# teticio/audio-diffusion

Measured on NVIDIA H100. Metric: mel-spectrograms/sec (1000-step DDPM, 256x256x1), higher is better.
Workload: dtype bf16 operands, fp32 accumulate (fp32 master weights, fp64 GroupNorm sums)

## Files before the change

### audio_diffusion_b200/_lib.py

```python
from __future__ import annotations

import ctypes as C
import os

_HERE = os.path.dirname(os.path.abspath(__file__))
LIB_PATH = os.environ.get("B200AD_LIB") or os.path.join(_HERE, "libb200ad.so")

MAX_BLOCKS = 8


class UNetConfigC(C.Structure):
    _fields_ = [
        ("in_channels", C.c_int), ("out_channels", C.c_int), ("layers_per_block", C.c_int), ("num_blocks", C.c_int),
        ("block_out_channels", C.c_int * MAX_BLOCKS), ("down_attn", C.c_int * MAX_BLOCKS),
        ("up_attn", C.c_int * MAX_BLOCKS), ("norm_num_groups", C.c_int), ("norm_eps", C.c_float),
        ("attention_head_dim", C.c_int), ("cross_attention_dim", C.c_int), ("down_cross", C.c_int * MAX_BLOCKS),
        ("up_cross", C.c_int * MAX_BLOCKS),
    ]


class VAEConfigC(C.Structure):
    _fields_ = [
        ("in_channels", C.c_int), ("out_channels", C.c_int), ("latent_channels", C.c_int), ("layers_per_block", C.c_int),
        ("num_blocks", C.c_int), ("block_out_channels", C.c_int * MAX_BLOCKS), ("norm_num_groups", C.c_int),
        ("norm_eps", C.c_float),
    ]


class OptimHParamsC(C.Structure):
    _fields_ = [("lr", C.c_float), ("beta1", C.c_float), ("beta2", C.c_float), ("eps", C.c_float),
                ("weight_decay", C.c_float), ("max_grad_norm", C.c_float), ("ema_decay", C.c_float), ("step", C.c_int)]


class StepCoefC(C.Structure):
    _fields_ = [("sqrt_1m_at", C.c_float), ("inv_sqrt_at", C.c_float), ("clip", C.c_float), ("c_x0", C.c_float),
                ("c_xt", C.c_float), ("c_eps", C.c_float), ("c_z", C.c_float), ("do_clip", C.c_int)]


class MelConfigC(C.Structure):
    _fields_ = [("x_res", C.c_int), ("y_res", C.c_int), ("sample_rate", C.c_int), ("n_fft", C.c_int),
                ("hop_length", C.c_int), ("top_db", C.c_int), ("n_iter", C.c_int)]


_VP, _SZ, _I = C.c_void_p, C.c_size_t, C.c_int
SYMBOLS = {
    "b200ad_last_error": (C.c_char_p, []),
    "b200ad_version": (_I, []),
    "b200ad_unet_create": (_I, [C.POINTER(UNetConfigC), C.POINTER(_VP)]),
    "b200ad_unet_destroy": (None, [_VP]),
    "b200ad_unet_num_params": (_I, [_VP]),
    "b200ad_unet_param_name": (C.c_char_p, [_VP, _I]),
    "b200ad_unet_param_shape": (_I, [_VP, _I, C.POINTER(C.c_int64)]),
    "b200ad_unet_packed_bytes": (_SZ, [_VP]),
    "b200ad_unet_workspace_bytes": (_SZ, [_VP, _I, _I, _I]),
    "b200ad_unet_set_params": (_I, [_VP, C.POINTER(_VP), _VP, _SZ, _VP]),
    "b200ad_unet_bind_workspace": (_I, [_VP, _VP, _SZ, _I, _I, _I, _VP]),
    "b200ad_unet_forward": (_I, [_VP, _VP, _VP, _VP, _VP]),
    "b200ad_unet_set_encoding": (_I, [_VP, _VP, _I]),
    "b200ad_unet_forward_step": (_I, [_VP, _VP, _VP, _VP, C.POINTER(StepCoefC), _VP, _VP, _VP]),
    "b200ad_unet_forward_step_dev": (_I, [_VP, _VP, _VP, _VP, _VP, _VP, _VP]),
    "b200ad_step_scalars_upload": (_I, [C.POINTER(StepCoefC), C.c_float, _VP, _VP, C.c_int, _VP]),
    "b200ad_unet_profile_step": (_I, [_VP, _VP, _VP, _VP, C.POINTER(StepCoefC), _VP, C.POINTER(C.c_float),
                                      C.POINTER(_I), C.POINTER(C.c_double), _I, _VP]),
    "b200ad_unet_debug_tensor": (_I, [_VP, C.c_char_p, _VP, C.POINTER(_I), _VP]),
    "b200ad_unet_last_launch_count": (_I, [_VP]),
    "b200ad_unet_conv_plan": (_I, [_VP, _I, _I, _I, _I, C.POINTER(_I), _I]),
    "b200ad_unet_set_training": (_I, [_VP, _I]),
    "b200ad_unet_grad_floats": (_SZ, [_VP]),
    "b200ad_unet_grad_offset": (_SZ, [_VP, _I]),
    "b200ad_unet_backward_bytes": (_SZ, [_VP]),
    "b200ad_unet_bind_backward": (_I, [_VP, _VP, _SZ, _VP, _VP]),
    "b200ad_unet_backward": (_I, [_VP, _VP, _VP, _I, _VP]),
    "b200ad_unet_backward_launch_count": (_I, [_VP]),
    "b200ad_unet_debug_grad": (_I, [_VP, C.c_char_p, _I, _VP, C.POINTER(_I), _VP]),
    "b200ad_vae_set_training": (_I, [_VP, _I]),
    "b200ad_vae_grad_floats": (_SZ, [_VP]),
    "b200ad_vae_grad_offset": (_SZ, [_VP, _I]),
    "b200ad_vae_backward_bytes": (_SZ, [_VP]),
    "b200ad_vae_bind_backward": (_I, [_VP, _VP, _SZ, _VP, _VP]),
    "b200ad_vae_decoder_backward": (_I, [_VP, _VP, _VP, _I, _VP]),
    "b200ad_vae_encoder_backward": (_I, [_VP, _VP, _VP, _I, _VP]),
    "b200ad_vae_backward_launch_count": (_I, [_VP]),
    "b200ad_vae_debug_grad": (_I, [_VP, C.c_char_p, _I, _VP, C.POINTER(_I), _VP]),
    "b200ad_vae_create": (_I, [C.POINTER(VAEConfigC), C.POINTER(_VP)]),
    "b200ad_vae_destroy": (None, [_VP]),
    "b200ad_vae_num_params": (_I, [_VP]),
    "b200ad_vae_param_name": (C.c_char_p, [_VP, _I]),
    "b200ad_vae_param_shape": (_I, [_VP, _I, C.POINTER(C.c_int64)]),
    "b200ad_vae_packed_bytes": (_SZ, [_VP]),
    "b200ad_vae_workspace_bytes": (_SZ, [_VP, _I, _I, _I]),
    "b200ad_vae_set_params": (_I, [_VP, C.POINTER(_VP), _VP, _SZ, _VP]),
    "b200ad_vae_bind_workspace": (_I, [_VP, _VP, _SZ, _I, _I, _I, _VP]),
    "b200ad_vae_encode": (_I, [_VP, _VP, _VP, _VP, _VP, _VP]),
    "b200ad_vae_decode": (_I, [_VP, _VP, _VP, _VP]),
    "b200ad_vae_debug_tensor": (_I, [_VP, C.c_char_p, _VP, C.POINTER(_I), _VP]),
    "b200ad_vae_last_launch_count": (_I, [_VP]),
    "b200ad_optim_create": (_I, [_I, C.POINTER(C.c_int64), C.POINTER(_VP), C.POINTER(_VP), C.POINTER(_VP),
                                C.POINTER(_VP), C.POINTER(_VP)]),
    "b200ad_optim_destroy": (None, [_VP]),
    "b200ad_optim_step": (_I, [_VP, C.POINTER(_VP), C.POINTER(OptimHParamsC), _VP, _VP]),
    "b200ad_mse_loss_grad": (_I, [_VP, _VP, _SZ, _VP, _VP, _VP, _VP]),
    "b200ad_conv2d_scratch_bytes": (_SZ, [_I] * 7),
    "b200ad_conv2d": (_I, [_VP] * 7 + [_I] * 7 + [_VP, _SZ, _VP]),
    "b200ad_conv2d_dgrad": (_I, [_VP, _VP, _VP] + [_I] * 6 + [_VP, _SZ, _VP]),
    "b200ad_conv2d_wgrad_scratch_bytes": (_SZ, [_I] * 5),
    "b200ad_conv2d_wgrad": (_I, [_VP, _VP, _VP] + [_I] * 6 + [_VP, _SZ, _VP]),
    "b200ad_gn_conv2d": (_I, [_VP, _VP, _VP, _I, C.c_float, _I, _VP, _VP, _VP] + [_I] * 6 + [_VP, _SZ, _VP]),
    "b200ad_group_norm": (_I, [_VP] * 4 + [_I] * 5 + [C.c_float, _I, _VP, _SZ, _VP]),
    "b200ad_mha_scratch_bytes": (_SZ, [_I] * 5),
    "b200ad_mha_forward_backward": (_I, [_VP] * 8 + [_I] * 5 + [_VP, _SZ, _VP]),
    "b200ad_mel_scratch_bytes": (_SZ, [C.POINTER(MelConfigC), _I]),
    "b200ad_mel_encode": (_I, [C.POINTER(MelConfigC), _VP, _VP, _VP, _I, _VP, _SZ, _VP]),
    "b200ad_mel_encode_ref": (_I, [C.POINTER(MelConfigC), _VP, _VP, _VP, _I, _VP, _VP, _VP, _SZ, _VP]),
    "b200ad_mel_decode": (_I, [C.POINTER(MelConfigC), _VP, _VP, _VP, _I, C.c_uint64, _VP, _SZ, _VP]),
    "b200ad_sample_to_u8": (_I, [_VP, _VP, _SZ, _VP]),
}

_lib = None


def lib() -> C.CDLL:
    global _lib
    if _lib is None:
        if not os.path.exists(LIB_PATH):
            raise RuntimeError(
                f"{LIB_PATH} is missing: build it with `python -c 'import __graft_entry__ as g; g.build()'` "
                "(there is no CPU fallback for the audio_diffusion_b200 hot path)")
        l = C.CDLL(LIB_PATH)
        for name, (res, args) in SYMBOLS.items():
            fn = getattr(l, name)
            fn.restype = res
            fn.argtypes = args
        _lib = l
    return _lib


class B200ADError(RuntimeError):
    pass


def check(status: int) -> None:
    if status != 0:
        raise B200ADError(lib().b200ad_last_error().decode())


def require_cuda():
    import torch

    if not torch.cuda.is_available():
        raise B200ADError("audio_diffusion_b200 needs a CUDA device (H100, sm_90a); there is no CPU fallback")


def stream_ptr():
    import torch

    return C.c_void_p(torch.cuda.current_stream().cuda_stream)
```

### audio_diffusion_b200/csrc/api.cu

```cuda
#include <cstdio>
#include <cstring>

#include "../../include/b200ad.h"
#include "bwd_kernels.cuh"
#include "taps.cuh"

namespace b200ad {
int set_err(const char* fmt, ...);
}
using namespace b200ad;

#define CK(call)                                                                      \
  do {                                                                                \
    cudaError_t e__ = (call);                                                         \
    if (e__ != cudaSuccess) return set_err("%s: %s", #call, cudaGetErrorString(e__)); \
  } while (0)

static size_t al(size_t x) { return (x + 255) & ~(size_t)255; }

struct ConvScratch {
  size_t x, par, res, out, wpack, ident, stats, instats, ss, total;
};
static ConvScratch conv_scratch_layout(int N, int cin, int cout, int H, int W, int K, int stride) {
  ConvScratch s{};
  const Geom gi = make_geom(N, H, W);
  const int Ho = stride > 0 ? H / stride : 2 * H, Wo = stride > 0 ? W / stride : 2 * W;
  const Geom go = make_geom(N, Ho, Wo);
  size_t off = 0;
  s.x = off; off = al(off + (size_t)N * (cin / 8) * gi.PL * 16);
  s.par = off; if (stride == 2) off = al(off + (size_t)4 * N * (cin / 8) * go.PL * 16);
  s.res = off; off = al(off + (size_t)N * (cout / 8) * go.PL * 16);
  s.out = off; off = al(off + (size_t)N * (cout / 8) * go.PL * 16);
  s.wpack = off; off = al(off + (size_t)(cout / 128) * (cin / 16) * (K * K > 16 ? K * K : 16) * CONV_B_TAP);
  s.ident = off; off = al(off + (size_t)(cout / 128) * (cout / 16) * CONV_B_TAP);
  s.stats = off; off = al(off + (size_t)N * (cout / 4) * 2 * sizeof(stat_t));
  s.instats = off; off = al(off + (size_t)N * (cin / 4) * 2 * sizeof(stat_t));
  s.ss = off; off = al(off + (size_t)N * cin * sizeof(float2));
  s.total = off;
  return s;
}

extern "C" size_t b200ad_conv2d_scratch_bytes(int N, int cin, int cout, int H, int W, int K, int stride) {
  return conv_scratch_layout(N, cin, cout, H, W, K, stride).total;
}

static int conv2d_impl(const float* x, const float* w, const float* bias, const float* temb, const float* residual,
                       float* y, float* stats_out, int N, int cin, int cout, int H, int W, int K, int stride,
                       const float* gn_gamma, const float* gn_beta, int gn_groups, float gn_eps, int gn_silu,
                       void* scratch, size_t scratch_bytes, void* stream) {
  if (cin % 16 || cout % 128) return set_err("conv2d: cin %% 16 and cout %% 128 must be 0");
  if (!((K == 3 || K == 1) && (stride == 1 || ((stride == 2 || stride == -2) && K == 3)))) return set_err("conv2d: unsupported K/stride");
  if (stride == -2 && (residual || gn_gamma || temb)) return set_err("conv2d: upsample form takes no residual / GroupNorm / temb");
  if (stride == 2 && (H % 2 || W % 2)) return set_err("conv2d: stride 2 needs even H, W");
  if (stride == 2 && (residual || gn_gamma)) return set_err("conv2d: residual / fused GroupNorm need stride 1");
  const ConvScratch L = conv_scratch_layout(N, cin, cout, H, W, K, stride);
  if (scratch_bytes < L.total) return set_err("conv2d: scratch too small");
  cudaStream_t st = (cudaStream_t)stream;
  uint8_t* sb = (uint8_t*)scratch;
  CK(cudaMemsetAsync(sb, 0, L.total, st));
  const int Ho = stride > 0 ? H / stride : 2 * H, Wo = stride > 0 ? W / stride : 2 * W;
  const Geom go = make_geom(N, Ho, Wo);
  __nv_bfloat16* xp = (__nv_bfloat16*)(sb + L.x);
  __nv_bfloat16* par = (__nv_bfloat16*)(sb + L.par);
  __nv_bfloat16* rp = (__nv_bfloat16*)(sb + L.res);
  __nv_bfloat16* op = (__nv_bfloat16*)(sb + L.out);
  __nv_bfloat16* wp = (__nv_bfloat16*)(sb + L.wpack);
  stat_t* stp = (stat_t*)(sb + L.stats);
  CK(launch_nchw_to_pf8(x, xp, N, cin, H, W, st));
  if (residual) CK(launch_nchw_to_pf8(residual, rp, N, cout, Ho, Wo, st));

  ConvParams p{};
  p.N = N; p.H = Ho; p.W = Wo; p.Wp = go.Wp; p.lead = go.lead; p.PL = go.PL;
  p.cout = cout;
  p.out = op; p.bias = bias; p.temb = temb; p.temb_stride = cout;
  p.stats = stats_out ? stp : nullptr;
  if (stride == 1) {
    const TapSet t = taps_conv(K);
    CK(launch_pack_weights(w, cout, cin, K, K, 0, cin / 16, t.pack, wp, st));
    ConvSeg& s = p.seg[0];
    set_seg(s, xp, cin / 8, cin, H, W, wp, t);
    p.nseg = 1;
    if (gn_gamma) {
      stat_t* ist = (stat_t*)(sb + L.instats);
      float2* ss = (float2*)(sb + L.ss);
      CK(launch_quad_stats(xp, ist, N, cin, H, W, st));
      GnApplyParams g{};
      g.src[0] = xp; g.stats[0] = ist; g.C[0] = cin; g.C[1] = 0; g.gamma = gn_gamma; g.beta = gn_beta;
      g.N = N; g.H = H; g.W = W; g.groups = gn_groups; g.eps = gn_eps;
      CK(launch_gn_finalize(g, ss, st));
      s.ss = ss; s.ss_stride = cin; s.silu = gn_silu;
    }
    if (residual) {
      __nv_bfloat16* ident = (__nv_bfloat16*)(sb + L.ident);
      CK(launch_pack_identity(cout, ident, st));
      set_seg(p.seg[1], rp, cout / 8, cout, Ho, Wo, ident, taps_conv(1));
      p.nseg = 2;
    }
  } else if (stride == 2) {
    CK(launch_parity_split(xp, par, N, cin, H, W, st));
    const size_t tsz = (size_t)N * (cin / 8) * go.PL * 8;
    size_t woff = 0;
    for (int a = 0; a < 2; ++a)
      for (int b = 0; b < 2; ++b) {
        const TapSet t = taps_parity(a, b);
        __nv_bfloat16* wseg = wp + woff / 2;
        CK(launch_pack_weights(w, cout, cin, 3, 3, 0, cin / 16, t.pack, wseg, st));
        woff += (size_t)(cout / 128) * (cin / 16) * t.pack.ntaps * CONV_B_TAP;
        set_seg(p.seg[a * 2 + b], par + (size_t)(a * 2 + b) * tsz, cin / 8, cin, Ho, Wo, wseg, t);
      }
    p.nseg = 4;
  }
  int dev = 0, sms = 132;
  CK(cudaGetDevice(&dev));
  CK(cudaDeviceGetAttribute(&sms, cudaDevAttrMultiProcessorCount, dev));
  if (stride == -2) {
    const Geom gi = make_geom(N, H, W);
    p.H = H; p.W = W; p.Wp = gi.Wp; p.lead = gi.lead; p.PL = gi.PL;
    p.up2 = 1;
    p.nseg = 1;
    size_t woff = 0;
    for (int pa = 0; pa < 2; ++pa)
      for (int pb = 0; pb < 2; ++pb) {
        const TapSet t = taps_up2(pa, pb);
        __nv_bfloat16* wseg = wp + woff / 2;
        CK(launch_pack_weights(w, cout, cin, 3, 3, 0, cin / 16, t.pack, wseg, st));
        woff += (size_t)(cout / 128) * (cin / 16) * 4 * CONV_B_TAP;
        set_seg(p.seg[0], xp, cin / 8, cin, H, W, wseg, t);
        p.oy = pa; p.ox = pb;
        CK(launch_conv_tc(p, sms, st));
      }
  } else {
    CK(launch_conv_tc(p, sms, st));
  }
  CK(launch_pf8_to_nchw(op, y, N, cout, Ho, Wo, st));
  if (stats_out) CK(launch_stats_to_float(stp, stats_out, N * (cout / 4) * 2, st));
  return 0;
}

extern "C" int b200ad_conv2d(const float* x, const float* w, const float* bias, const float* temb, const float* residual,
                             float* y, float* stats_out, int N, int cin, int cout, int H, int W, int K, int stride,
                             void* scratch, size_t scratch_bytes, void* stream) {
  return conv2d_impl(x, w, bias, temb, residual, y, stats_out, N, cin, cout, H, W, K, stride, nullptr, nullptr, 0, 0.f, 0,
                     scratch, scratch_bytes, stream);
}

extern "C" int b200ad_conv2d_dgrad(const float* gy, const float* w, float* gx, int N, int cin, int cout, int H, int W, int K,
                                   void* scratch, size_t scratch_bytes, void* stream) {
  if (cout % 16 || cin % 128) return set_err("conv2d_dgrad: cout %% 16 and cin %% 128 must be 0");
  if (K != 3 && K != 1) return set_err("conv2d_dgrad: K must be 1 or 3");
  const ConvScratch L = conv_scratch_layout(N, cout, cin, H, W, K, 1);
  if (scratch_bytes < L.total) return set_err("conv2d_dgrad: scratch too small");
  cudaStream_t st = (cudaStream_t)stream;
  uint8_t* sb = (uint8_t*)scratch;
  CK(cudaMemsetAsync(sb, 0, L.total, st));
  const Geom g = make_geom(N, H, W);
  __nv_bfloat16* gyp = (__nv_bfloat16*)(sb + L.x);
  __nv_bfloat16* gxp = (__nv_bfloat16*)(sb + L.out);
  __nv_bfloat16* wp = (__nv_bfloat16*)(sb + L.wpack);
  CK(launch_nchw_to_pf8(gy, gyp, N, cout, H, W, st));
  const TapSet t = taps_mirrored(K);
  CK(launch_pack_weights(w, cin, cin, K, K, 0, cout / 16, t.pack, wp, st, cin));
  ConvParams p{};
  p.N = N; p.H = H; p.W = W; p.Wp = g.Wp; p.lead = g.lead; p.PL = g.PL;
  p.cout = cin;
  p.out = gxp; p.bias = nullptr; p.temb = nullptr; p.temb_stride = 0; p.stats = nullptr;
  set_seg(p.seg[0], gyp, cout / 8, cout, H, W, wp, t);
  p.nseg = 1;
  int dev = 0, sms = 132;
  CK(cudaGetDevice(&dev));
  CK(cudaDeviceGetAttribute(&sms, cudaDevAttrMultiProcessorCount, dev));
  CK(launch_conv_tc(p, sms, st));
  CK(launch_pf8_to_nchw(gxp, gx, N, cin, H, W, st));
  return 0;
}

extern "C" int b200ad_conv2d_wgrad(const float* gy, const float* a, float* dw, int N, int cin, int cout, int H, int W, int K,
                                   void* scratch, size_t scratch_bytes, void* stream) {
  if (cout % 128 || cin % 32) return set_err("conv2d_wgrad: cout %% 128 and cin %% 32 must be 0");
  if (K != 3 && K != 1) return set_err("conv2d_wgrad: K must be 1 or 3");
  const Geom g = make_geom(N, H, W);
  const size_t gyb = al((size_t)N * (cout / 8) * g.PL * 16), ab = al((size_t)N * (cin / 8) * g.PL * 16);
  if (scratch_bytes < gyb + ab) return set_err("conv2d_wgrad: scratch too small (%zu < %zu)", scratch_bytes, gyb + ab);
  cudaStream_t st = (cudaStream_t)stream;
  uint8_t* sb = (uint8_t*)scratch;
  CK(cudaMemsetAsync(sb, 0, gyb + ab, st));
  __nv_bfloat16* gyp = (__nv_bfloat16*)sb;
  __nv_bfloat16* ap = (__nv_bfloat16*)(sb + gyb);
  CK(launch_nchw_to_pf8(gy, gyp, N, cout, H, W, st));
  CK(launch_nchw_to_pf8(a, ap, N, cin, H, W, st));
  CK(cudaMemsetAsync(dw, 0, (size_t)cout * cin * K * K * sizeof(float), st));
  int dev = 0, sms = 132;
  CK(cudaGetDevice(&dev));
  CK(cudaDeviceGetAttribute(&sms, cudaDevAttrMultiProcessorCount, dev));
  WgradDesc d{};
  d.gy = gyp; d.act = ap; d.dw = dw; d.N = N; d.H = H; d.W = W; d.cout = cout; d.cin = cin;
  d.gy_img_planes = cout / 8; d.act_img_planes = cin / 8; d.cin_total = cin; d.ci_off = 0; d.ntaps_total = K * K;
  const TapSet t = taps_conv(K);
  d.ntaps = K * K;
  for (int k = 0; k < K * K; ++k) { d.dh[k] = t.dh[k]; d.dw_[k] = t.dw[k]; d.tapidx[k] = t.wtap[k]; }
  CK(launch_wgrad_tc(d, sms, st));
  return 0;
}
extern "C" size_t b200ad_conv2d_wgrad_scratch_bytes(int N, int cin, int cout, int H, int W) {
  const Geom g = make_geom(N, H, W);
  return al((size_t)N * (cout / 8) * g.PL * 16) + al((size_t)N * (cin / 8) * g.PL * 16);
}

extern "C" int b200ad_gn_conv2d(const float* x, const float* gamma, const float* beta, int groups, float eps, int silu,
                                const float* w, const float* bias, float* y, int N, int cin, int cout, int H, int W, int K,
                                void* scratch, size_t scratch_bytes, void* stream) {
  if (!gamma || !beta) return set_err("gn_conv2d: gamma and beta are required");
  return conv2d_impl(x, w, bias, nullptr, nullptr, y, nullptr, N, cin, cout, H, W, K, 1, gamma, beta, groups, eps, silu,
                     scratch, scratch_bytes, stream);
}

extern "C" int b200ad_group_norm(const float* x, const float* gamma, const float* beta, float* y, int N, int C, int H,
                                 int W, int groups, float eps, int silu, void* scratch, size_t scratch_bytes, void* stream) {
  if (C % 32) return set_err("group_norm: C %% 32 != 0");
  const Geom g = make_geom(N, H, W);
  const size_t tb = al((size_t)N * (C / 8) * g.PL * 16);
  const size_t need = 2 * tb + al((size_t)N * (C / 4) * 2 * sizeof(stat_t));
  if (scratch_bytes < need) return set_err("group_norm: scratch too small (%zu < %zu)", scratch_bytes, need);
  cudaStream_t st = (cudaStream_t)stream;
  uint8_t* sb = (uint8_t*)scratch;
  CK(cudaMemsetAsync(sb, 0, need, st));
  __nv_bfloat16* xp = (__nv_bfloat16*)sb;
  __nv_bfloat16* yp = (__nv_bfloat16*)(sb + tb);
  stat_t* stats = (stat_t*)(sb + 2 * tb);
  CK(launch_nchw_to_pf8(x, xp, N, C, H, W, st));
  CK(launch_quad_stats(xp, stats, N, C, H, W, st));
  GnApplyParams p{};
  p.src[0] = xp; p.stats[0] = stats; p.C[0] = C; p.src[1] = nullptr; p.stats[1] = nullptr; p.C[1] = 0;
  p.gamma = gamma; p.beta = beta; p.dst = yp; p.N = N; p.H = H; p.W = W; p.groups = groups; p.eps = eps; p.silu = silu;
  CK(launch_gn_apply(p, st));
  CK(launch_pf8_to_nchw(yp, y, N, C, H, W, st));
  return 0;
}

struct MhaScratch {
  size_t qkv_f, qkv, o, go, gqkv, lse, dsum, total;
};
static MhaScratch mha_scratch_layout(int N, int C, int heads, int H, int W) {
  MhaScratch s{};
  const Geom g = make_geom(N, H, W);
  const size_t pf = (size_t)N * (C / 8) * g.PL * 16, rows = (size_t)N * heads * H * W * sizeof(float);
  size_t off = 0;
  s.qkv_f = off; off = al(off + (size_t)N * 3 * C * H * W * sizeof(float));
  s.qkv = off; off = al(off + 3 * pf);
  s.o = off; off = al(off + pf);
  s.go = off; off = al(off + pf);
  s.gqkv = off; off = al(off + 3 * pf);
  s.lse = off; off = al(off + rows);
  s.dsum = off; off = al(off + rows);
  s.total = off;
  return s;
}
extern "C" size_t b200ad_mha_scratch_bytes(int N, int C, int heads, int H, int W) {
  return mha_scratch_layout(N, C, heads, H, W).total;
}
extern "C" int b200ad_mha_forward_backward(const float* q, const float* k, const float* v, const float* dout, float* out,
                                           float* dq, float* dk, float* dv, int N, int C, int heads, int H, int W,
                                           void* scratch, size_t scratch_bytes, void* stream) {
  if (heads < 1 || C % heads || (C / heads != 16 && C / heads != 32 && C / heads != 64))
    return set_err("mha_forward_backward: head_dim C / heads must be 16, 32 or 64");
  const MhaScratch L = mha_scratch_layout(N, C, heads, H, W);
  if (scratch_bytes < L.total) return set_err("mha_forward_backward: scratch too small (%zu < %zu)", scratch_bytes, L.total);
  cudaStream_t st = (cudaStream_t)stream;
  uint8_t* sb = (uint8_t*)scratch;
  CK(cudaMemsetAsync(sb, 0, L.total, st));
  float* qkvf = (float*)(sb + L.qkv_f);
  __nv_bfloat16* qkv = (__nv_bfloat16*)(sb + L.qkv);
  __nv_bfloat16* o = (__nv_bfloat16*)(sb + L.o);
  __nv_bfloat16* go = (__nv_bfloat16*)(sb + L.go);
  __nv_bfloat16* gqkv = (__nv_bfloat16*)(sb + L.gqkv);
  const size_t img = (size_t)C * H * W * sizeof(float);
  const float* src[3] = {q, k, v};
  for (int j = 0; j < 3; ++j)
    CK(cudaMemcpy2DAsync((uint8_t*)qkvf + j * img, 3 * img, src[j], img, img, N, cudaMemcpyDeviceToDevice, st));
  CK(launch_nchw_to_pf8(qkvf, qkv, N, 3 * C, H, W, st));
  CK(launch_nchw_to_pf8(dout, go, N, C, H, W, st));
  CK(launch_mha_flash(qkv, o, N, C, heads, H, W, st, (float*)(sb + L.lse)));
  CK(launch_mha_bwd(qkv, o, go, (const float*)(sb + L.lse), (float*)(sb + L.dsum), gqkv, N, C, heads, H, W, st));
  CK(launch_pf8_to_nchw(o, out, N, C, H, W, st));
  CK(launch_pf8_to_nchw(gqkv, qkvf, N, 3 * C, H, W, st));
  float* dst[3] = {dq, dk, dv};
  for (int j = 0; j < 3; ++j)
    CK(cudaMemcpy2DAsync(dst[j], img, (const uint8_t*)qkvf + j * img, 3 * img, img, N, cudaMemcpyDeviceToDevice, st));
  return 0;
}

extern "C" int b200ad_sample_to_u8(const float* x, uint8_t* img, size_t n, void* stream) {
  CK(launch_sample_to_u8(x, img, n, (cudaStream_t)stream));
  return 0;
}
```

### audio_diffusion_b200/csrc/common.cuh

```cuda
#pragma once
#include <cuda_bf16.h>
#include <cuda_runtime.h>
#include <stdint.h>
#include <stdio.h>

namespace b200ad {

typedef double stat_t;

struct Geom {
  int N, H, W, Wp, lead, PL;
};
__host__ __device__ inline Geom make_geom(int N, int H, int W) {
  Geom g;
  g.N = N; g.H = H; g.W = W; g.Wp = W + 1; g.lead = g.Wp + 8;
  g.PL = g.lead + H * g.Wp + g.Wp + 8 + 512;
  return g;
}

#ifdef __CUDACC__
__device__ __forceinline__ uint32_t smem_u32(const void* p) {
  return static_cast<uint32_t>(__cvta_generic_to_shared(p));
}
__device__ __forceinline__ void mbar_init(uint32_t bar, uint32_t count) {
  asm volatile("mbarrier.init.shared::cta.b64 [%0], %1;" ::"r"(bar), "r"(count));
}
__device__ __forceinline__ void mbar_fence_init() {
  asm volatile("fence.mbarrier_init.release.cluster;" ::: "memory");
}
__device__ __forceinline__ void mbar_arrive_expect_tx(uint32_t bar, uint32_t bytes) {
  asm volatile("mbarrier.arrive.expect_tx.shared::cta.b64 _, [%0], %1;" ::"r"(bar), "r"(bytes) : "memory");
}
__device__ __forceinline__ void mbar_arrive(uint32_t bar) {
  asm volatile("mbarrier.arrive.shared::cta.b64 _, [%0];" ::"r"(bar) : "memory");
}
__device__ __forceinline__ bool mbar_try_wait(uint32_t bar, uint32_t parity) {
  uint32_t ok;
  asm volatile(
      "{\n\t.reg .pred p;\n\t"
      "mbarrier.try_wait.parity.shared::cta.b64 p, [%1], %2;\n\t"
      "selp.u32 %0, 1, 0, p;\n\t}"
      : "=r"(ok) : "r"(bar), "r"(parity) : "memory");
  return ok != 0;
}
__device__ __forceinline__ void mbar_wait(uint32_t bar, uint32_t parity) {
  if (mbar_try_wait(bar, parity)) return;
  long long t0 = clock64();
  while (!mbar_try_wait(bar, parity)) {
    if (clock64() - t0 > 4000000000LL) __trap();
  }
}

__device__ __forceinline__ void mbar_wait_warp(uint32_t bar, uint32_t parity) {
  if (__all_sync(0xffffffffu, mbar_try_wait(bar, parity))) return;
  long long t0 = clock64();
  while (!__all_sync(0xffffffffu, mbar_try_wait(bar, parity))) {
    if (clock64() - t0 > 4000000000LL) {
      if ((threadIdx.x & 31) == 0) printf("b200ad: mbarrier timeout (block %d warp %d bar %u parity %u)\n", blockIdx.x, threadIdx.x >> 5, bar, parity);
      __trap();
    }
  }
}

__device__ __forceinline__ void bulk_g2s(uint32_t dst_smem, const void* src, uint32_t bytes, uint32_t bar) {
  asm volatile(
      "cp.async.bulk.shared::cluster.global.mbarrier::complete_tx::bytes [%0], [%1], %2, [%3];"
      ::"r"(dst_smem), "l"(src), "r"(bytes), "r"(bar) : "memory");
}

__device__ __forceinline__ void bulk_s2g(void* dst, uint32_t src_smem, uint32_t bytes) {
  asm volatile("cp.async.bulk.global.shared::cta.bulk_group [%0], [%1], %2;" ::"l"(dst), "r"(src_smem), "r"(bytes) : "memory");
}
__device__ __forceinline__ void bulk_commit() { asm volatile("cp.async.bulk.commit_group;" ::: "memory"); }
__device__ __forceinline__ void bulk_wait_read_all() { asm volatile("cp.async.bulk.wait_group.read 0;" ::: "memory"); }
__device__ __forceinline__ void bulk_wait_all() { asm volatile("cp.async.bulk.wait_group 0;" ::: "memory"); }
__device__ __forceinline__ void named_bar_sync(int id, int nthreads) {
  asm volatile("bar.sync %0, %1;" ::"r"(id), "r"(nthreads) : "memory");
}

__device__ __forceinline__ void tensor_g2s_5d(uint32_t dst_smem, const void* tmap, int c0, int c1, int c2, int c3, int c4,
                                              uint32_t bar) {
  asm volatile(
      "cp.async.bulk.tensor.5d.shared::cluster.global.tile.mbarrier::complete_tx::bytes [%0], [%1, {%2, %3, %4, %5, %6}], [%7];"
      ::"r"(dst_smem), "l"(tmap), "r"(c0), "r"(c1), "r"(c2), "r"(c3), "r"(c4), "r"(bar) : "memory");
}
__device__ __forceinline__ void tensor_s2g_5d(const void* tmap, int c0, int c1, int c2, int c3, int c4, uint32_t src_smem) {
  asm volatile("cp.async.bulk.tensor.5d.global.shared::cta.tile.bulk_group [%0, {%1, %2, %3, %4, %5}], [%6];"
               ::"l"(tmap), "r"(c0), "r"(c1), "r"(c2), "r"(c3), "r"(c4), "r"(src_smem) : "memory");
}

__device__ __forceinline__ void tensor_g2s_4d(uint32_t dst_smem, const void* tmap, int c0, int c1, int c2, int c3, uint32_t bar) {
  asm volatile(
      "cp.async.bulk.tensor.4d.shared::cluster.global.tile.mbarrier::complete_tx::bytes [%0], [%1, {%2, %3, %4, %5}], [%6];"
      ::"r"(dst_smem), "l"(tmap), "r"(c0), "r"(c1), "r"(c2), "r"(c3), "r"(bar) : "memory");
}
__device__ __forceinline__ void tensor_s2g_4d(const void* tmap, int c0, int c1, int c2, int c3, uint32_t src_smem) {
  asm volatile("cp.async.bulk.tensor.4d.global.shared::cta.tile.bulk_group [%0, {%1, %2, %3, %4}], [%5];"
               ::"l"(tmap), "r"(c0), "r"(c1), "r"(c2), "r"(c3), "r"(src_smem) : "memory");
}

__device__ __forceinline__ void bulk_prefetch_l2(const void* src, uint32_t bytes) {
  asm volatile("cp.async.bulk.prefetch.L2.global [%0], %1;" ::"l"(src), "r"(bytes) : "memory");
}

__device__ __forceinline__ uint64_t gmma_desc(uint32_t saddr, uint32_t lbo_bytes, uint32_t sbo_bytes) {
  uint64_t d = 0;
  d |= (uint64_t)((saddr >> 4) & 0x3FFF);
  d |= (uint64_t)((lbo_bytes >> 4) & 0x3FFF) << 16;
  d |= (uint64_t)((sbo_bytes >> 4) & 0x3FFF) << 32;
  return d;
}
__device__ __forceinline__ void wgmma_fence() { asm volatile("wgmma.fence.sync.aligned;" ::: "memory"); }
__device__ __forceinline__ void wgmma_commit() { asm volatile("wgmma.commit_group.sync.aligned;" ::: "memory"); }
template <int N>
__device__ __forceinline__ void wgmma_wait() { asm volatile("wgmma.wait_group.sync.aligned %0;" ::"n"(N) : "memory"); }

template <int TA, int TB>
__device__ __forceinline__ void wgmma_m64n32k16(float* d, uint64_t a, uint64_t b) {
  asm volatile(
      "{\n\t.reg .pred p;\n\tsetp.ne.b32 p, %18, 0;\n\t"
      "wgmma.mma_async.sync.aligned.m64n32k16.f32.bf16.bf16 {"
      "%0, %1, %2, %3, %4, %5, %6, %7, %8, %9, %10, %11, %12, %13, %14, %15"
      "}, %16, %17, p, 1, 1, %19, %20;\n\t}"
      : "+f"(d[0]), "+f"(d[1]), "+f"(d[2]), "+f"(d[3]), "+f"(d[4]), "+f"(d[5]), "+f"(d[6]), "+f"(d[7]),
        "+f"(d[8]), "+f"(d[9]), "+f"(d[10]), "+f"(d[11]), "+f"(d[12]), "+f"(d[13]), "+f"(d[14]), "+f"(d[15])
      : "l"(a), "l"(b), "r"(1), "n"(TA), "n"(TB));
}
template <int TA, int TB>
__device__ __forceinline__ void wgmma_m64n64k16(float* d, uint64_t a, uint64_t b) {
  asm volatile(
      "{\n\t.reg .pred p;\n\tsetp.ne.b32 p, %34, 0;\n\t"
      "wgmma.mma_async.sync.aligned.m64n64k16.f32.bf16.bf16 {"
      "%0, %1, %2, %3, %4, %5, %6, %7, %8, %9, %10, %11, %12, %13, %14, %15, "
      "%16, %17, %18, %19, %20, %21, %22, %23, %24, %25, %26, %27, %28, %29, %30, %31"
      "}, %32, %33, p, 1, 1, %35, %36;\n\t}"
      : "+f"(d[0]), "+f"(d[1]), "+f"(d[2]), "+f"(d[3]), "+f"(d[4]), "+f"(d[5]), "+f"(d[6]), "+f"(d[7]),
        "+f"(d[8]), "+f"(d[9]), "+f"(d[10]), "+f"(d[11]), "+f"(d[12]), "+f"(d[13]), "+f"(d[14]), "+f"(d[15]),
        "+f"(d[16]), "+f"(d[17]), "+f"(d[18]), "+f"(d[19]), "+f"(d[20]), "+f"(d[21]), "+f"(d[22]), "+f"(d[23]),
        "+f"(d[24]), "+f"(d[25]), "+f"(d[26]), "+f"(d[27]), "+f"(d[28]), "+f"(d[29]), "+f"(d[30]), "+f"(d[31])
      : "l"(a), "l"(b), "r"(1), "n"(TA), "n"(TB));
}
template <int TA, int TB>
__device__ __forceinline__ void wgmma_m64n128k16(float* d, uint64_t a, uint64_t b) {
  asm volatile(
      "{\n\t.reg .pred p;\n\tsetp.ne.b32 p, %66, 0;\n\t"
      "wgmma.mma_async.sync.aligned.m64n128k16.f32.bf16.bf16 {"
      "%0, %1, %2, %3, %4, %5, %6, %7, %8, %9, %10, %11, %12, %13, %14, %15, "
      "%16, %17, %18, %19, %20, %21, %22, %23, %24, %25, %26, %27, %28, %29, %30, %31, "
      "%32, %33, %34, %35, %36, %37, %38, %39, %40, %41, %42, %43, %44, %45, %46, %47, "
      "%48, %49, %50, %51, %52, %53, %54, %55, %56, %57, %58, %59, %60, %61, %62, %63"
      "}, %64, %65, p, 1, 1, %67, %68;\n\t}"
      : "+f"(d[0]), "+f"(d[1]), "+f"(d[2]), "+f"(d[3]), "+f"(d[4]), "+f"(d[5]), "+f"(d[6]), "+f"(d[7]),
        "+f"(d[8]), "+f"(d[9]), "+f"(d[10]), "+f"(d[11]), "+f"(d[12]), "+f"(d[13]), "+f"(d[14]), "+f"(d[15]),
        "+f"(d[16]), "+f"(d[17]), "+f"(d[18]), "+f"(d[19]), "+f"(d[20]), "+f"(d[21]), "+f"(d[22]), "+f"(d[23]),
        "+f"(d[24]), "+f"(d[25]), "+f"(d[26]), "+f"(d[27]), "+f"(d[28]), "+f"(d[29]), "+f"(d[30]), "+f"(d[31]),
        "+f"(d[32]), "+f"(d[33]), "+f"(d[34]), "+f"(d[35]), "+f"(d[36]), "+f"(d[37]), "+f"(d[38]), "+f"(d[39]),
        "+f"(d[40]), "+f"(d[41]), "+f"(d[42]), "+f"(d[43]), "+f"(d[44]), "+f"(d[45]), "+f"(d[46]), "+f"(d[47]),
        "+f"(d[48]), "+f"(d[49]), "+f"(d[50]), "+f"(d[51]), "+f"(d[52]), "+f"(d[53]), "+f"(d[54]), "+f"(d[55]),
        "+f"(d[56]), "+f"(d[57]), "+f"(d[58]), "+f"(d[59]), "+f"(d[60]), "+f"(d[61]), "+f"(d[62]), "+f"(d[63])
      : "l"(a), "l"(b), "r"(1), "n"(TA), "n"(TB));
}
template <int TA, int TB>
__device__ __forceinline__ void wgmma_m64n256k16(float* d, uint64_t a, uint64_t b) {
  asm volatile(
      "{\n\t.reg .pred p;\n\tsetp.ne.b32 p, %130, 0;\n\t"
      "wgmma.mma_async.sync.aligned.m64n256k16.f32.bf16.bf16 {"
      "%0, %1, %2, %3, %4, %5, %6, %7, %8, %9, %10, %11, %12, %13, %14, %15, "
      "%16, %17, %18, %19, %20, %21, %22, %23, %24, %25, %26, %27, %28, %29, %30, %31, "
      "%32, %33, %34, %35, %36, %37, %38, %39, %40, %41, %42, %43, %44, %45, %46, %47, "
      "%48, %49, %50, %51, %52, %53, %54, %55, %56, %57, %58, %59, %60, %61, %62, %63, "
      "%64, %65, %66, %67, %68, %69, %70, %71, %72, %73, %74, %75, %76, %77, %78, %79, "
      "%80, %81, %82, %83, %84, %85, %86, %87, %88, %89, %90, %91, %92, %93, %94, %95, "
      "%96, %97, %98, %99, %100, %101, %102, %103, %104, %105, %106, %107, %108, %109, %110, %111, "
      "%112, %113, %114, %115, %116, %117, %118, %119, %120, %121, %122, %123, %124, %125, %126, %127"
      "}, %128, %129, p, 1, 1, %131, %132;\n\t}"
      : "+f"(d[0]), "+f"(d[1]), "+f"(d[2]), "+f"(d[3]), "+f"(d[4]), "+f"(d[5]), "+f"(d[6]), "+f"(d[7]),
        "+f"(d[8]), "+f"(d[9]), "+f"(d[10]), "+f"(d[11]), "+f"(d[12]), "+f"(d[13]), "+f"(d[14]), "+f"(d[15]),
        "+f"(d[16]), "+f"(d[17]), "+f"(d[18]), "+f"(d[19]), "+f"(d[20]), "+f"(d[21]), "+f"(d[22]), "+f"(d[23]),
        "+f"(d[24]), "+f"(d[25]), "+f"(d[26]), "+f"(d[27]), "+f"(d[28]), "+f"(d[29]), "+f"(d[30]), "+f"(d[31]),
        "+f"(d[32]), "+f"(d[33]), "+f"(d[34]), "+f"(d[35]), "+f"(d[36]), "+f"(d[37]), "+f"(d[38]), "+f"(d[39]),
        "+f"(d[40]), "+f"(d[41]), "+f"(d[42]), "+f"(d[43]), "+f"(d[44]), "+f"(d[45]), "+f"(d[46]), "+f"(d[47]),
        "+f"(d[48]), "+f"(d[49]), "+f"(d[50]), "+f"(d[51]), "+f"(d[52]), "+f"(d[53]), "+f"(d[54]), "+f"(d[55]),
        "+f"(d[56]), "+f"(d[57]), "+f"(d[58]), "+f"(d[59]), "+f"(d[60]), "+f"(d[61]), "+f"(d[62]), "+f"(d[63]),
        "+f"(d[64]), "+f"(d[65]), "+f"(d[66]), "+f"(d[67]), "+f"(d[68]), "+f"(d[69]), "+f"(d[70]), "+f"(d[71]),
        "+f"(d[72]), "+f"(d[73]), "+f"(d[74]), "+f"(d[75]), "+f"(d[76]), "+f"(d[77]), "+f"(d[78]), "+f"(d[79]),
        "+f"(d[80]), "+f"(d[81]), "+f"(d[82]), "+f"(d[83]), "+f"(d[84]), "+f"(d[85]), "+f"(d[86]), "+f"(d[87]),
        "+f"(d[88]), "+f"(d[89]), "+f"(d[90]), "+f"(d[91]), "+f"(d[92]), "+f"(d[93]), "+f"(d[94]), "+f"(d[95]),
        "+f"(d[96]), "+f"(d[97]), "+f"(d[98]), "+f"(d[99]), "+f"(d[100]), "+f"(d[101]), "+f"(d[102]), "+f"(d[103]),
        "+f"(d[104]), "+f"(d[105]), "+f"(d[106]), "+f"(d[107]), "+f"(d[108]), "+f"(d[109]), "+f"(d[110]), "+f"(d[111]),
        "+f"(d[112]), "+f"(d[113]), "+f"(d[114]), "+f"(d[115]), "+f"(d[116]), "+f"(d[117]), "+f"(d[118]), "+f"(d[119]),
        "+f"(d[120]), "+f"(d[121]), "+f"(d[122]), "+f"(d[123]), "+f"(d[124]), "+f"(d[125]), "+f"(d[126]), "+f"(d[127])
      : "l"(a), "l"(b), "r"(1), "n"(TA), "n"(TB));
}
__device__ __forceinline__ void wgmma_m64n128k16_x2(float* d, uint64_t a, uint64_t b0, uint64_t b1) {
  asm volatile(
      "{\n\t.reg .pred p;\n\tsetp.ne.b32 p, %131, 0;\n\t"
      "wgmma.mma_async.sync.aligned.m64n128k16.f32.bf16.bf16 {"
      "%0, %1, %2, %3, %4, %5, %6, %7, %8, %9, %10, %11, %12, %13, %14, %15, "
      "%16, %17, %18, %19, %20, %21, %22, %23, %24, %25, %26, %27, %28, %29, %30, %31, "
      "%32, %33, %34, %35, %36, %37, %38, %39, %40, %41, %42, %43, %44, %45, %46, %47, "
      "%48, %49, %50, %51, %52, %53, %54, %55, %56, %57, %58, %59, %60, %61, %62, %63"
      "}, %128, %129, p, 1, 1, 0, 0;\n\t"
      "wgmma.mma_async.sync.aligned.m64n128k16.f32.bf16.bf16 {"
      "%64, %65, %66, %67, %68, %69, %70, %71, %72, %73, %74, %75, %76, %77, %78, %79, "
      "%80, %81, %82, %83, %84, %85, %86, %87, %88, %89, %90, %91, %92, %93, %94, %95, "
      "%96, %97, %98, %99, %100, %101, %102, %103, %104, %105, %106, %107, %108, %109, %110, %111, "
      "%112, %113, %114, %115, %116, %117, %118, %119, %120, %121, %122, %123, %124, %125, %126, %127"
      "}, %128, %130, p, 1, 1, 0, 0;\n\t}"
      : "+f"(d[0]), "+f"(d[1]), "+f"(d[2]), "+f"(d[3]), "+f"(d[4]), "+f"(d[5]), "+f"(d[6]), "+f"(d[7]),
        "+f"(d[8]), "+f"(d[9]), "+f"(d[10]), "+f"(d[11]), "+f"(d[12]), "+f"(d[13]), "+f"(d[14]), "+f"(d[15]),
        "+f"(d[16]), "+f"(d[17]), "+f"(d[18]), "+f"(d[19]), "+f"(d[20]), "+f"(d[21]), "+f"(d[22]), "+f"(d[23]),
        "+f"(d[24]), "+f"(d[25]), "+f"(d[26]), "+f"(d[27]), "+f"(d[28]), "+f"(d[29]), "+f"(d[30]), "+f"(d[31]),
        "+f"(d[32]), "+f"(d[33]), "+f"(d[34]), "+f"(d[35]), "+f"(d[36]), "+f"(d[37]), "+f"(d[38]), "+f"(d[39]),
        "+f"(d[40]), "+f"(d[41]), "+f"(d[42]), "+f"(d[43]), "+f"(d[44]), "+f"(d[45]), "+f"(d[46]), "+f"(d[47]),
        "+f"(d[48]), "+f"(d[49]), "+f"(d[50]), "+f"(d[51]), "+f"(d[52]), "+f"(d[53]), "+f"(d[54]), "+f"(d[55]),
        "+f"(d[56]), "+f"(d[57]), "+f"(d[58]), "+f"(d[59]), "+f"(d[60]), "+f"(d[61]), "+f"(d[62]), "+f"(d[63]),
        "+f"(d[64]), "+f"(d[65]), "+f"(d[66]), "+f"(d[67]), "+f"(d[68]), "+f"(d[69]), "+f"(d[70]), "+f"(d[71]),
        "+f"(d[72]), "+f"(d[73]), "+f"(d[74]), "+f"(d[75]), "+f"(d[76]), "+f"(d[77]), "+f"(d[78]), "+f"(d[79]),
        "+f"(d[80]), "+f"(d[81]), "+f"(d[82]), "+f"(d[83]), "+f"(d[84]), "+f"(d[85]), "+f"(d[86]), "+f"(d[87]),
        "+f"(d[88]), "+f"(d[89]), "+f"(d[90]), "+f"(d[91]), "+f"(d[92]), "+f"(d[93]), "+f"(d[94]), "+f"(d[95]),
        "+f"(d[96]), "+f"(d[97]), "+f"(d[98]), "+f"(d[99]), "+f"(d[100]), "+f"(d[101]), "+f"(d[102]), "+f"(d[103]),
        "+f"(d[104]), "+f"(d[105]), "+f"(d[106]), "+f"(d[107]), "+f"(d[108]), "+f"(d[109]), "+f"(d[110]), "+f"(d[111]),
        "+f"(d[112]), "+f"(d[113]), "+f"(d[114]), "+f"(d[115]), "+f"(d[116]), "+f"(d[117]), "+f"(d[118]), "+f"(d[119]),
        "+f"(d[120]), "+f"(d[121]), "+f"(d[122]), "+f"(d[123]), "+f"(d[124]), "+f"(d[125]), "+f"(d[126]), "+f"(d[127])
      : "l"(a), "l"(b0), "l"(b1), "r"(1));
}

__device__ __forceinline__ bool elect_one() {
  uint32_t pred;
  asm volatile(
      "{\n\t.reg .pred p;\n\t"
      "elect.sync _|p, 0xffffffff;\n\t"
      "selp.u32 %0, 1, 0, p;\n\t}"
      : "=r"(pred));
  return pred != 0;
}

__device__ __forceinline__ void fence_proxy_async_smem() { asm volatile("fence.proxy.async.shared::cta;" ::: "memory"); }

__device__ __forceinline__ float tanh_approx(float x) {
  float y;
  asm("tanh.approx.f32 %0, %1;" : "=f"(y) : "f"(x));
  return y;
}
__device__ __forceinline__ float silu_tanh(float x) { return x * fmaf(0.5f, tanh_approx(0.5f * x), 0.5f); }
__device__ __forceinline__ float silu_f(float x) { return x / (1.0f + __expf(-x)); }
__device__ __forceinline__ uint32_t pack_bf16x2(float lo, float hi) {
  __nv_bfloat162 v = __floats2bfloat162_rn(lo, hi);
  return *reinterpret_cast<uint32_t*>(&v);
}
__device__ __forceinline__ float2 unpack_bf16x2(uint32_t u) {
  __nv_bfloat162 v = *reinterpret_cast<__nv_bfloat162*>(&u);
  return __bfloat1622float2(v);
}

typedef float2 f32x2_t;
__device__ __forceinline__ f32x2_t f2_pack(float lo, float hi) { return make_float2(lo, hi); }
__device__ __forceinline__ float2 f2_unpack(f32x2_t v) { return v; }
__device__ __forceinline__ f32x2_t f2_add(f32x2_t a, f32x2_t b) { return make_float2(a.x + b.x, a.y + b.y); }
__device__ __forceinline__ f32x2_t f2_fma(f32x2_t a, f32x2_t b, f32x2_t c) {
  return make_float2(fmaf(a.x, b.x, c.x), fmaf(a.y, b.y, c.y));
}
__device__ __forceinline__ f32x2_t f2_from_bf16x2(uint32_t u) {
  return f2_pack(__uint_as_float(u << 16), __uint_as_float(u & 0xffff0000u));
}
__device__ __forceinline__ uint32_t f2_to_bf16x2(f32x2_t v) {
  uint32_t r;
  asm("cvt.rn.bf16x2.f32 %0, %1, %2;" : "=r"(r) : "f"(v.y), "f"(v.x));
  return r;
}

__device__ __forceinline__ void stmatrix_x4_trans(uint32_t saddr, uint32_t r0, uint32_t r1, uint32_t r2, uint32_t r3) {
  asm volatile("stmatrix.sync.aligned.m8n8.x4.trans.shared.b16 [%0], {%1, %2, %3, %4};"
               ::"r"(saddr), "r"(r0), "r"(r1), "r"(r2), "r"(r3) : "memory");
}

__device__ __forceinline__ void mma_bf16_16x8x16(float (&c)[4], uint32_t a0, uint32_t a1, uint32_t a2, uint32_t a3, uint32_t b0,
                                                 uint32_t b1) {
  asm volatile("mma.sync.aligned.m16n8k16.row.col.f32.bf16.bf16.f32 {%0,%1,%2,%3}, {%4,%5,%6,%7}, {%8,%9}, {%0,%1,%2,%3};"
               : "+f"(c[0]), "+f"(c[1]), "+f"(c[2]), "+f"(c[3]) : "r"(a0), "r"(a1), "r"(a2), "r"(a3), "r"(b0), "r"(b1));
}

__device__ __forceinline__ long long pf8_pixel(const Geom& g, int p, int W) {
  return (long long)(g.lead + (p / W) * g.Wp + (p % W)) * 8;
}
#endif

}
```

### audio_diffusion_b200/csrc/conv_tc.cu

```cuda
#include <cuda.h>
#include <cudaTypedefs.h>

#include <cstdlib>

#include "conv_tc.cuh"

namespace b200ad {

struct alignas(64) ConvMaps {
  CUtensorMap src[CONV_MAXSEG];
  CUtensorMap out;
};

__host__ __device__ __forceinline__ int window_pixels(const ConvParams& p, const ConvSeg& sg, int G) {
  return p.tile2d ? (p.tw + sg.hl + sg.hr) * (p.th + sg.ht + sg.hb)
                  : G * CONV_TM + (sg.ht + sg.hb) * p.Wp + sg.hl + sg.hr;
}
__host__ __device__ __forceinline__ int window_pitch(const ConvParams& p, const ConvSeg& sg) {
  return p.tile2d ? p.tw + sg.hl + sg.hr : p.Wp;
}

constexpr int CONV_THREADS = 384;
constexpr int CONV_XF_THREADS = 64;
constexpr int CONV_SPLANE = CONV_MAXG * CONV_TM * 16;
constexpr int CONV_STG_WG = 8 * CONV_SPLANE;
constexpr int CONV_STAGING = 2 * CONV_STG_WG;
static size_t conv_smem_bytes(const ConvParams& p) {
  return (size_t)p.as * p.a_stage + (size_t)p.bs * CONV_B_SLOT + CONV_STAGING + 1024;
}

struct WorkItem {
  int n, ntile, m0, G;
  int r0, c0;
};

__device__ __forceinline__ WorkItem decode_work(const ConvParams& p, int w) {
  WorkItem wi;
  wi.ntile = w % p.ntiles_n;
  const int gidx = w / p.ntiles_n;
  if (p.tile2d) {
    wi.n = gidx / p.groups_per_img;
    const int t = gidx - wi.n * p.groups_per_img, tx = t / p.tiles_y;
    wi.r0 = (t - tx * p.tiles_y) * p.th;
    wi.c0 = tx * p.tw;
    wi.m0 = 0;
    wi.G = CONV_MAXG;
    return wi;
  }
  wi.r0 = wi.c0 = 0;
  if (p.pack) {
    wi.n = gidx * p.pack;
    wi.m0 = 0;
    wi.G = min(p.pack, p.N - wi.n);
    return wi;
  }
  wi.n = gidx / p.groups_per_img;
  const int g = gidx - wi.n * p.groups_per_img;
  wi.m0 = g * (CONV_MAXG * CONV_TM);
  const int rem = p.H * p.Wp - wi.m0;
  wi.G = min(CONV_MAXG, (rem + CONV_TM - 1) / CONV_TM);
  return wi;
}

template <bool SILU>
__device__ __forceinline__ uint4 xform_vec(uint4 v, const f32x2_t (&sc)[4], const f32x2_t (&sh)[4]) {
  uint32_t u[4] = {v.x, v.y, v.z, v.w};
#pragma unroll
  for (int e = 0; e < 4; ++e) {
    f32x2_t a = f2_fma(f2_from_bf16x2(u[e]), sc[e], sh[e]);
    if (SILU) {
      const float2 f = f2_unpack(a);
      a = f2_fma(a, f2_pack(tanh_approx(f.x), tanh_approx(f.y)), a);
    }
    u[e] = f2_to_bf16x2(a);
  }
  return make_uint4(u[0], u[1], u[2], u[3]);
}

template <bool SQUARE>
__global__ void __launch_bounds__(CONV_THREADS, 1) conv_tc_kernel(const __grid_constant__ ConvParams p,
                                                                  const __grid_constant__ ConvMaps maps) {
  constexpr int ASM = CONV_AS_MAX, BSM = CONV_BS_MAX;
  const int AS = p.as;
  const int BS = p.bs;
  extern __shared__ __align__(128) uint8_t smem[];
  const int warp = __shfl_sync(0xffffffffu, (int)(threadIdx.x >> 5), 0);
  const int lane = threadIdx.x & 31;
  const int a_bytes = p.a_stage;

  uint8_t* bring = smem + AS * a_bytes;
  uint8_t* stg = bring + BS * CONV_B_SLOT;
  uint8_t* ctrl = stg + CONV_STAGING;
  uint64_t* bars = reinterpret_cast<uint64_t*>(ctrl);
  const uint32_t smem_base = smem_u32(smem);
  const uint32_t bring_base = smem_u32(bring);
  const uint32_t bar_fullA = smem_u32(bars);
  const uint32_t bar_readyA = smem_u32(bars + ASM);
  const uint32_t bar_emptyA = smem_u32(bars + 2 * ASM);
  const uint32_t bar_fullB = smem_u32(bars + 3 * ASM);
  const uint32_t bar_emptyB = smem_u32(bars + 3 * ASM + BSM);
  static_assert((3 * ASM + 2 * BSM) * 8 <= 1024, "barrier block overflows");

  if (warp == 1 && lane == 0) {
    for (int s = 0; s < AS; ++s) {
      mbar_init(bar_fullA + 8 * s, 1);
      mbar_init(bar_readyA + 8 * s, CONV_XF_THREADS / 32);
      mbar_init(bar_emptyA + 8 * s, 8);
    }
    for (int s = 0; s < BS; ++s) {
      mbar_init(bar_fullB + 8 * s, 1);
      mbar_init(bar_emptyB + 8 * s, 8);
    }
    mbar_fence_init();
  }
  __syncthreads();

  asm volatile("griddepcontrol.launch_dependents;" ::: "memory");
  if (warp != 1) asm volatile("griddepcontrol.wait;" ::: "memory");

  if (warp == 0) {
    int stage = 0;
    uint32_t phase = 0;
    for (int w = blockIdx.x; w < p.total_work; w += gridDim.x) {
      const WorkItem wi = decode_work(p, w);
      for (int s = 0; s < p.nseg; ++s) {
        const ConvSeg& sg = p.seg[s];
        const uint32_t row_bytes = (uint32_t)window_pixels(p, sg, wi.G) * 16u;
        for (int ks = 0; ks < sg.ksteps; ++ks) {
          const uint32_t full = bar_fullA + 8 * stage;
          if (lane == 0) {
            mbar_wait(bar_emptyA + 8 * stage, phase ^ 1);
            mbar_arrive_expect_tx(full, 2u * row_bytes);
          }
          __syncwarp();
          const long long plane = (long long)(2 * ks + (lane & 1)) * p.PL;
          if (p.tile2d) {
            if (lane == 0)
              tensor_g2s_4d(smem_base + stage * a_bytes, &maps.src[s], 8 * (wi.c0 - sg.hl), wi.r0 - sg.ht, 2 * ks, wi.n, full);
          } else if (!p.pack) {
            const int pix0 = p.lead + wi.m0 - sg.ht * p.Wp - sg.hl;
            if (lane < 2)
              bulk_g2s(smem_base + stage * a_bytes + (uint32_t)lane * row_bytes,
                       sg.src + (long long)wi.n * sg.img_stride + (plane + pix0) * 8, row_bytes, full);
          } else {
            const int g = lane >> 1, lead_px = sg.ht * p.Wp + sg.hl, trail_px = sg.hb * p.Wp + sg.hr;
            const int cnt = CONV_TM + (g == 0 ? lead_px : 0) + (g == wi.G - 1 ? trail_px : 0);
            const int doff = (g == 0) ? 0 : lead_px + g * CONV_TM;
            const int pix0 = p.lead - (g == 0 ? lead_px : 0);
            if (g < wi.G && lane < 2 * CONV_MAXG)
              bulk_g2s(smem_base + stage * a_bytes + (uint32_t)(lane & 1) * row_bytes + (uint32_t)doff * 16u,
                       sg.src + (long long)(wi.n + g) * sg.img_stride + (plane + pix0) * 8, (uint32_t)cnt * 16u, full);
          }
          if (++stage == AS) { stage = 0; phase ^= 1; }
        }
      }
    }
  } else if (warp == 1) {
    if (lane == 0) {
      int stage = 0;
      uint32_t phase = 0;
      for (int w = blockIdx.x; w < p.total_work; w += gridDim.x) {
        const int ntile = w % p.ntiles_n;
        for (int s = 0; s < p.nseg; ++s) {
          const ConvSeg& sg = p.seg[s];
          const char* src = reinterpret_cast<const char*>(sg.wpack + (long long)ntile * sg.wtile_stride);
          for (int ks = 0; ks < sg.ksteps; ++ks) {
            for (int t0 = 0; t0 < sg.ntaps; t0 += CONV_BT) {
              const uint32_t bytes = (uint32_t)min(CONV_BT, sg.ntaps - t0) * CONV_B_TAP;
              mbar_wait(bar_emptyB + 8 * stage, phase ^ 1);
              if (p.dbg & 32) {
                mbar_arrive(bar_fullB + 8 * stage);
              } else {
                mbar_arrive_expect_tx(bar_fullB + 8 * stage, bytes);
                bulk_g2s(bring_base + stage * CONV_B_SLOT, src, bytes, bar_fullB + 8 * stage);
              }
              src += bytes;
              if (++stage == BS) { stage = 0; phase ^= 1; }
            }
          }
        }
      }
    }
  } else if (warp >= 4) {
    const int cw = (warp - 4) >> 2, wq = warp & 3, tid = threadIdx.x & 127;
    const uint32_t stg_w = smem_u32(stg) + (uint32_t)(cw * CONV_STG_WG);
    const uint32_t st_addr = stg_w + (uint32_t)((2 * wq + ((lane >> 3) & 1)) * CONV_SPLANE + (8 * (lane >> 4) + (lane & 7)) * 16);
    const Geom og = make_geom(p.N, p.up2 ? 2 * p.H : p.H, p.up2 ? 2 * p.W : p.W);
    const long long out_img_stride = (long long)(p.cout >> 3) * og.PL * 8;
    const int hw_end = p.H * p.Wp;
    const bool do_stats = p.stats != nullptr;
    const bool issuer = tid < 8 * CONV_MAXG;
    float acc[CONV_MAXG * CONV_TM / 2];
    int sa = 0, sb = 0;
    uint32_t pa = 0, pb = 0;
    for (int w = blockIdx.x; w < p.total_work; w += gridDim.x) {
      const WorkItem wi = decode_work(p, w);
#pragma unroll
      for (int i = 0; i < CONV_MAXG * CONV_TM / 2; ++i) acc[i] = 0.f;
      int pend_b = -1, pend_a = -1;
      auto release = [&]() {
        __syncwarp();
        if (lane == 0) {
          if (pend_b >= 0) mbar_arrive(bar_emptyB + 8 * pend_b);
          if (pend_a >= 0) mbar_arrive(bar_emptyA + 8 * pend_a);
        }
      };
      for (int s = 0, ks = 0; s < p.nseg;) {
        const ConvSeg& sg = p.seg[s];
        const uint32_t xlbo = (uint32_t)window_pixels(p, sg, wi.G) * 16u;
        const uint32_t xsbo = p.tile2d ? (uint32_t)window_pitch(p, sg) * 16u : 128u;
        const int ntaps = sg.ntaps;
        mbar_wait(bar_readyA + 8 * sa, pa);
        const uint32_t abase = smem_base + sa * a_bytes;
        for (int t0 = 0; t0 < ntaps; t0 += CONV_BT) {
          mbar_wait(bar_fullB + 8 * sb, pb);
          const uint32_t bbase = bring_base + sb * CONV_B_SLOT + (uint32_t)(cw * 1024);
          const int nt = min(CONV_BT, ntaps - t0);
          wgmma_fence();
          for (int t = 0; t < nt; ++t) {
            const uint64_t wdesc = gmma_desc(bbase + (uint32_t)t * CONV_B_TAP, (CONV_NT / 8) * 128, 128);
            const uint64_t xdesc = gmma_desc(abase + (uint32_t)sg.aoff[t0 + t] * 16u, xlbo, xsbo);
            if constexpr (SQUARE) {
              wgmma_m64n128k16_x2(acc, wdesc, xdesc, xdesc + (128u >> 4));
            } else if (wi.G == 2) {
              wgmma_m64n256k16<0, 0>(acc, wdesc, xdesc);
            } else {
              wgmma_m64n128k16<0, 0>(acc, wdesc, xdesc);
            }
          }
          wgmma_commit();
          wgmma_wait<1>();
          release();
          pend_b = sb;
          pend_a = (t0 + CONV_BT >= ntaps) ? sa : -1;
          if (++sb == BS) { sb = 0; pb ^= 1; }
        }
        if (++sa == AS) { sa = 0; pa ^= 1; }
        if (++ks == sg.ksteps) { ks = 0; ++s; }
      }
      wgmma_wait<0>();
      release();

      if (issuer) bulk_wait_read_all();
      named_bar_sync(1 + cw, 128);
      if (!(p.dbg & 8)) {
        float ssum[2] = {0.f, 0.f}, ssq[2] = {0.f, 0.f};
#pragma unroll
        for (int g = 0; g < CONV_MAXG; ++g) {
          if (g < wi.G) {
            const int n = p.pack ? wi.n + g : wi.n;
            float bias[2];
#pragma unroll
            for (int h = 0; h < 2; ++h) {
              const int c = wi.ntile * CONV_NT + cw * 64 + wq * 16 + 8 * h + (lane >> 2);
              bias[h] = p.bias ? __ldg(p.bias + c) : 0.f;
              if (p.temb) bias[h] += __ldg(p.temb + (long long)n * p.temb_stride + c);
            }
            int m = (p.pack ? 0 : wi.m0 + g * CONV_TM) + 2 * (lane & 3);
            int col = m % p.Wp;
#pragma unroll
            for (int k = 0; k < CONV_TM / 16; ++k) {
              uint32_t pk[4];
#pragma unroll
              for (int u = 0; u < 2; ++u) {
                const int col1 = (col + 1 == p.Wp) ? 0 : col + 1;
                const bool v0 = p.tile2d || (m < hw_end && col < p.W), v1 = p.tile2d || (m + 1 < hw_end && col1 < p.W);
#pragma unroll
                for (int h = 0; h < 2; ++h) {
                  const int j = g * (CONV_TM / 8) + 2 * k + u;
                  const float a0 = v0 ? acc[4 * j + 2 * h] + bias[h] : 0.f;
                  const float a1 = v1 ? acc[4 * j + 2 * h + 1] + bias[h] : 0.f;
                  ssum[h] += a0 + a1;
                  ssq[h] = fmaf(a0, a0, fmaf(a1, a1, ssq[h]));
                  pk[2 * u + h] = pack_bf16x2(a0, a1);
                }
                m += 8;
                col += 8;
                while (col >= p.Wp) col -= p.Wp;
              }
              stmatrix_x4_trans(st_addr + (uint32_t)((g * CONV_TM + 16 * k) * 16), pk[0], pk[1], pk[2], pk[3]);
            }
            if (do_stats && (p.pack || g == wi.G - 1)) {
#pragma unroll
              for (int h = 0; h < 2; ++h) {
                float s1 = ssum[h], s2 = ssq[h];
#pragma unroll
                for (int o = 1; o < 16; o <<= 1) {
                  s1 += __shfl_xor_sync(0xffffffffu, s1, o);
                  s2 += __shfl_xor_sync(0xffffffffu, s2, o);
                }
                if ((lane & 15) == 0) {
                  const int c = wi.ntile * CONV_NT + cw * 64 + wq * 16 + 8 * h + (lane >> 2);
                  stat_t* sdst = p.stats + ((long long)n * (p.cout >> 2) + (c >> 2)) * 2;
                  atomicAdd(sdst, (stat_t)s1);
                  atomicAdd(sdst + 1, (stat_t)s2);
                }
                ssum[h] = 0.f;
                ssq[h] = 0.f;
              }
            }
          }
        }
      }
      if (p.tile2d) {
        fence_proxy_async_smem();
        named_bar_sync(1 + cw, 128);
        if (SQUARE) {
          const int g = tid >> 3, pl = tid & 7;
          if (issuer && !(p.dbg & 2)) {
            const uint32_t src = stg_w + (uint32_t)(pl * CONV_SPLANE + g * CONV_TM * 16);
            const int c = wi.c0 + 8 * g, plane = wi.ntile * 16 + cw * 8 + pl;
            if (p.up2) tensor_s2g_5d(&maps.out, 0, c, wi.r0, plane, wi.n, src);
            else       tensor_s2g_4d(&maps.out, 8 * c, wi.r0, plane, wi.n, src);
            bulk_commit();
          }
        } else if (tid == 0 && !(p.dbg & 2)) {
          tensor_s2g_4d(&maps.out, 8 * wi.c0, wi.r0, wi.ntile * 16 + cw * 8, wi.n, stg_w);
          bulk_commit();
        }
      } else if (!p.up2) {
        fence_proxy_async_smem();
        named_bar_sync(1 + cw, 128);
        const int g = tid >> 3, pl = tid & 7;
        if (issuer && g < wi.G && !(p.dbg & 2)) {
          const int n = p.pack ? wi.n + g : wi.n;
          bulk_s2g(p.out + (long long)n * out_img_stride + (long long)(wi.ntile * 16 + cw * 8 + pl) * og.PL * 8 +
                       (long long)(p.lead + (p.pack ? 0 : wi.m0 + CONV_TM * g)) * 8,
                   stg_w + (uint32_t)(pl * CONV_SPLANE + g * CONV_TM * 16), (uint32_t)CONV_TM * 16u);
          bulk_commit();
        }
      } else {
        named_bar_sync(1 + cw, 128);
        const int npx = wi.G * CONV_TM;
        for (int i = tid; i < 8 * npx && !(p.dbg & 2); i += 128) {
          const int pl = i / npx, px = i - pl * npx, g = px >> 7;
          const int m = p.pack ? px & (CONV_TM - 1) : wi.m0 + px;
          const int hh = m / p.Wp, ww = m - hh * p.Wp;
          if (m < hw_end && ww < p.W) {
            const int n = p.pack ? wi.n + g : wi.n;
            const uint4 o = *reinterpret_cast<const uint4*>(stg + cw * CONV_STG_WG + pl * CONV_SPLANE + px * 16);
            *reinterpret_cast<uint4*>(p.out + (long long)n * out_img_stride + (long long)(wi.ntile * 16 + cw * 8 + pl) * og.PL * 8 +
                                      (long long)(og.lead + (2 * hh + p.oy) * og.Wp + 2 * ww + p.ox) * 8) = o;
          }
        }
      }
    }
    if (issuer) bulk_wait_all();
  } else {
    const int tidx = (warp - 2) * 32 + lane;
    int stage = 0;
    uint32_t phase = 0;
    for (int w = blockIdx.x; w < p.total_work; w += gridDim.x) {
      const WorkItem wi = decode_work(p, w);
      for (int s = 0; s < p.nseg; ++s) {
        const ConvSeg& sg = p.seg[s];
        const int npix = window_pixels(p, sg, wi.G);
        const int pitch = window_pitch(p, sg);
        const float2* ssn = sg.ss ? sg.ss + (long long)wi.n * sg.ss_stride : nullptr;
        const int cbase = p.tile2d ? wi.c0 - sg.hl : 0;
        int row0, col0;
        if (p.tile2d) {
          row0 = wi.r0 - sg.ht + tidx / pitch;
          col0 = tidx - (tidx / pitch) * pitch;
        } else {
          const int m_first = wi.m0 - sg.ht * p.Wp - sg.hl + tidx;
          row0 = (m_first >= 0) ? m_first / p.Wp : -1 - ((-1 - m_first) / p.Wp);
          col0 = m_first - row0 * p.Wp;
        }
        const int drow = CONV_XF_THREADS / pitch;
        const int dcol = CONV_XF_THREADS - drow * pitch;
        const bool silu = sg.silu != 0;
        for (int ks = 0; ks < sg.ksteps; ++ks) {
          f32x2_t sc0[4], sh0[4], sc1[4], sh1[4];
          if (ssn && !p.pack) {
            const float4* sp = reinterpret_cast<const float4*>(ssn + ks * 16);
            const float hs = silu ? 0.5f : 1.0f;
#pragma unroll
            for (int e = 0; e < 4; ++e) {
              const float4 a = __ldg(sp + e), b = __ldg(sp + 4 + e);
              sc0[e] = f2_pack(a.x * hs, a.z * hs); sh0[e] = f2_pack(a.y * hs, a.w * hs);
              sc1[e] = f2_pack(b.x * hs, b.z * hs); sh1[e] = f2_pack(b.y * hs, b.w * hs);
            }
          }
          mbar_wait(bar_fullA + 8 * stage, phase);
          if (ssn && p.pack && !(p.dbg & 64)) {
            uint4* base = reinterpret_cast<uint4*>(smem + stage * a_bytes);
            const int lead_px = sg.ht * p.Wp + sg.hl, hw = p.H * p.Wp;
            const float hs = silu ? 0.5f : 1.0f;
            for (int g = 0; g < wi.G; ++g) {
              const float4* sp = reinterpret_cast<const float4*>(ssn + (long long)g * sg.ss_stride + ks * 16);
#pragma unroll
              for (int e = 0; e < 4; ++e) {
                const float4 a = __ldg(sp + e), b = __ldg(sp + 4 + e);
                sc0[e] = f2_pack(a.x * hs, a.z * hs); sh0[e] = f2_pack(a.y * hs, a.w * hs);
                sc1[e] = f2_pack(b.x * hs, b.z * hs); sh1[e] = f2_pack(b.y * hs, b.w * hs);
              }
              for (int m = tidx; m < hw; m += CONV_XF_THREADS) {
                const int r = m / p.Wp;
                const int px = lead_px + g * CONV_TM + m;
                uint4 a = make_uint4(0, 0, 0, 0), b = make_uint4(0, 0, 0, 0);
                if (m - r * p.Wp < p.W) {
                  a = base[px];
                  b = base[npix + px];
                  if (silu) { a = xform_vec<true>(a, sc0, sh0); b = xform_vec<true>(b, sc1, sh1); }
                  else      { a = xform_vec<false>(a, sc0, sh0); b = xform_vec<false>(b, sc1, sh1); }
                }
                base[px] = a;
                base[npix + px] = b;
              }
            }
            fence_proxy_async_smem();
          } else if (ssn && !(p.dbg & 64)) {
            uint4* base = reinterpret_cast<uint4*>(smem + stage * a_bytes);
            int row = row0, col = col0;
            for (int px = tidx; px < npix; px += CONV_XF_THREADS) {
              const bool valid = (row >= 0) && (row < p.H) && ((unsigned)(cbase + col) < (unsigned)p.W);
              uint4 a = make_uint4(0, 0, 0, 0), b = make_uint4(0, 0, 0, 0);
              if (valid) {
                a = base[px];
                b = base[npix + px];
                if (silu) { a = xform_vec<true>(a, sc0, sh0); b = xform_vec<true>(b, sc1, sh1); }
                else      { a = xform_vec<false>(a, sc0, sh0); b = xform_vec<false>(b, sc1, sh1); }
              }
              base[px] = a;
              base[npix + px] = b;
              row += drow; col += dcol;
              if (col >= pitch) { col -= pitch; ++row; }
            }
            fence_proxy_async_smem();
          }
          __syncwarp();
          if (lane == 0) mbar_arrive(bar_readyA + 8 * stage);
          if (++stage == AS) { stage = 0; phase ^= 1; }
        }
      }
    }
  }

  if (p.fin.ss) __threadfence();
  __syncthreads();

  if (p.fin.ss) {
    __shared__ unsigned s_last;
    if (threadIdx.x == 0) {
      __threadfence();
      s_last = (atomicAdd(p.fin.counter, 1u) == gridDim.x - 1) ? 1u : 0u;
    }
    __syncthreads();
    if (s_last) {
      __threadfence();
      const ConvGnFin& f = p.fin;
      const int Ct = f.C[0] + f.C[1], cpg = Ct / f.groups;
      float* gmean = reinterpret_cast<float*>(smem);
      float* grstd = gmean + p.N * f.groups;
      const double cnt = (double)cpg * (double)f.HW;
      for (int i = threadIdx.x; i < p.N * f.groups; i += CONV_THREADS) {
        const int n = i / f.groups, gi = i - n * f.groups;
        double sm = 0., sq = 0.;
        for (int c0 = gi * cpg; c0 < (gi + 1) * cpg; c0 += 32) {
          double2 v[8];
#pragma unroll
          for (int k = 0; k < 8; ++k) {
            const int c = c0 + 4 * k;
            v[k] = make_double2(0., 0.);
            if (c < (gi + 1) * cpg) {
              const stat_t* st = (c < f.C[0]) ? f.stats[0] + ((long long)n * (f.C[0] >> 2) + (c >> 2)) * 2
                                              : f.stats[1] + ((long long)n * (f.C[1] >> 2) + ((c - f.C[0]) >> 2)) * 2;
              v[k] = __ldcg(reinterpret_cast<const double2*>(st));
            }
          }
#pragma unroll
          for (int k = 0; k < 8; ++k) { sm += v[k].x; sq += v[k].y; }
        }
        const double mean = sm / cnt;
        gmean[i] = (float)mean;
        grstd[i] = (float)(1.0 / sqrt(fmax(sq / cnt - mean * mean, 0.) + (double)f.eps));
      }
      __syncthreads();
      {
        const int total = p.N * Ct;
        const int dn = CONV_THREADS / Ct, dc = CONV_THREADS - dn * Ct;
        const float inv_cpg = 1.0f / (float)cpg;
        int i = threadIdx.x;
        int n = i / Ct, c = i - n * Ct;
        for (; i < total; i += CONV_THREADS) {
          const int gi = n * f.groups + (int)(((float)c + 0.5f) * inv_cpg);
          const float sc = __ldg(f.gamma + c) * grstd[gi];
          f.ss[i] = make_float2(sc, __ldg(f.beta + c) - gmean[gi] * sc);
          n += dn;
          c += dc;
          if (c >= Ct) { c -= Ct; ++n; }
        }
      }
      if (threadIdx.x == 0) *f.counter = 0u;
    }
  }
}

static cudaError_t encode_pf8_map(CUtensorMap* m, const __nv_bfloat16* base, const ConvParams& p, int cs, int rs, long long pl,
                                  int planes, long long img_stride, int bw, int bh, int bplanes) {
  static PFN_cuTensorMapEncodeTiled_v12000 encode = nullptr;
  if (!encode) {
    void* fn = nullptr;
    cudaDriverEntryPointQueryResult q;
    cudaError_t e = cudaGetDriverEntryPointByVersion("cuTensorMapEncodeTiled", &fn, 12000, cudaEnableDefault, &q);
    if (e != cudaSuccess) return e;
    if (q != cudaDriverEntryPointSuccess || !fn) return cudaErrorNotSupported;
    encode = reinterpret_cast<PFN_cuTensorMapEncodeTiled_v12000>(fn);
  }
  const cuuint32_t estride[5] = {1, 1, 1, 1, 1};
  CUresult r;
  if (cs == 1) {
    const cuuint64_t dim[4] = {(cuuint64_t)p.W * 8, (cuuint64_t)p.H, (cuuint64_t)planes, (cuuint64_t)p.N};
    const cuuint64_t stride[3] = {(cuuint64_t)rs * 16, (cuuint64_t)pl * 16, (cuuint64_t)img_stride * 2};
    const cuuint32_t box[4] = {(cuuint32_t)bw * 8, (cuuint32_t)bh, (cuuint32_t)bplanes, 1};
    r = encode(m, CU_TENSOR_MAP_DATA_TYPE_BFLOAT16, 4, (void*)base, dim, stride, box, estride, CU_TENSOR_MAP_INTERLEAVE_NONE,
               CU_TENSOR_MAP_SWIZZLE_NONE, CU_TENSOR_MAP_L2_PROMOTION_L2_256B, CU_TENSOR_MAP_FLOAT_OOB_FILL_NONE);
  } else {
    const cuuint64_t dim[5] = {8, (cuuint64_t)p.W, (cuuint64_t)p.H, (cuuint64_t)planes, (cuuint64_t)p.N};
    const cuuint64_t stride[4] = {(cuuint64_t)cs * 16, (cuuint64_t)rs * 16, (cuuint64_t)pl * 16, (cuuint64_t)img_stride * 2};
    const cuuint32_t box[5] = {8, (cuuint32_t)bw, (cuuint32_t)bh, (cuuint32_t)bplanes, 1};
    r = encode(m, CU_TENSOR_MAP_DATA_TYPE_BFLOAT16, 5, (void*)base, dim, stride, box, estride, CU_TENSOR_MAP_INTERLEAVE_NONE,
               CU_TENSOR_MAP_SWIZZLE_NONE, CU_TENSOR_MAP_L2_PROMOTION_L2_256B, CU_TENSOR_MAP_FLOAT_OOB_FILL_NONE);
  }
  return r == CUDA_SUCCESS ? cudaSuccess : cudaErrorInvalidValue;
}

int conv_dbg_env() {
  const char* dbg_env = getenv("B200AD_CONV_DBG");
  return dbg_env ? atoi(dbg_env) : 0;
}

cudaError_t plan_conv_tc(ConvParams& p, int num_sms) {
  if (p.nseg < 1 || p.nseg > CONV_MAXSEG) return cudaErrorInvalidValue;
  for (int s = 0; s < p.nseg; ++s) {
    ConvSeg& sg = p.seg[s];
    if (sg.ntaps > CONV_MAXTAPS || sg.ksteps < 1) return cudaErrorInvalidValue;
    if (sg.wtile_stride == 0) sg.wtile_stride = (long long)sg.ksteps * sg.ntaps * (CONV_B_TAP / 2);
    sg.ht = sg.hb = sg.hl = sg.hr = 0;
    for (int t = 0; t < sg.ntaps; ++t) {
      sg.ht |= sg.dh[t] < 0; sg.hb |= sg.dh[t] > 0;
      sg.hl |= sg.dw[t] < 0; sg.hr |= sg.dw[t] > 0;
    }
  }
  p.tile2d = 0;
  p.tw = p.th = 0;
  p.tiles_y = 0;
  p.groups_per_img = (p.H * p.Wp + CONV_MAXG * CONV_TM - 1) / (CONV_MAXG * CONV_TM);
  p.ntiles_n = p.cout / CONV_NT;
  p.total_work = p.N * p.groups_per_img * p.ntiles_n;
  p.pack = 0;
  int fits = 1;
  for (int s = 0; s < p.nseg; ++s) {
    const ConvSeg& sg = p.seg[s];
    if (p.H * p.Wp + sg.hb * p.Wp + sg.hr > CONV_TM || sg.ht * p.Wp + sg.hl > CONV_TM) fits = 0;
  }
  if (fits) {
    int best = 1;
    long long best_cost = -1;
    for (int g = 1; g <= CONV_MAXG; g *= 2) {
      const long long items = (long long)((p.N + g - 1) / g) * p.ntiles_n;
      const long long cost = ((items + num_sms - 1) / num_sms) * g;
      if (best_cost < 0 || cost <= best_cost) { best_cost = cost; best = g; }
    }
    p.pack = best;
    p.total_work = ((p.N + best - 1) / best) * p.ntiles_n;
  }
  const int tiles_img = (p.H * p.Wp + CONV_TM - 1) / CONV_TM;
  const int max_g = p.pack ? p.pack : (tiles_img < CONV_MAXG ? tiles_img : CONV_MAXG);
  if (!p.pack && !(p.dbg & 4096)) {
    auto window_cost = [&](const ConvParams& q, int G) {
      long long c = 0;
      for (int s = 0; s < q.nseg; ++s) c += (long long)window_pixels(q, q.seg[s], G) * q.seg[s].ksteps;
      return c;
    };
    long long best[3] = {(long long)tiles_img * CONV_TM, p.groups_per_img, 0};
    for (int i = 0; i < p.groups_per_img; ++i) best[2] += window_cost(p, min(CONV_MAXG, tiles_img - CONV_MAXG * i));
    const int shapes[2][2] = {{8, 32}, {16, 16}};
    for (const auto& sh : shapes) {
      const int tw = sh[0], th = sh[1];
      if (p.W % tw || p.H % th) continue;
      if (tw == 16 && p.H >= 64 && p.H % 32 == 0 && p.W % 8 == 0) continue;
      if (tw == 8 && p.up2) continue;
      ConvParams q = p;
      q.tile2d = 1; q.tw = tw; q.th = th;
      const long long items = (long long)(p.W / tw) * (p.H / th);
      const long long c[3] = {items * CONV_MAXG * CONV_TM, items, items * window_cost(q, CONV_MAXG)};
      if (c[0] < best[0] || (c[0] == best[0] && (c[1] < best[1] || (c[1] == best[1] && c[2] < best[2])))) {
        best[0] = c[0]; best[1] = c[1]; best[2] = c[2];
        p.tile2d = 1; p.tw = tw; p.th = th;
      }
    }
    if (p.tile2d) {
      p.tiles_y = p.H / p.th;
      p.groups_per_img = (p.W / p.tw) * p.tiles_y;
      p.total_work = p.N * p.groups_per_img * p.ntiles_n;
    }
  }
  int a_stage = 0;
  for (int s = 0; s < p.nseg; ++s) {
    const ConvSeg& sg = p.seg[s];
    const int npix = window_pixels(p, sg, max_g), pitch = window_pitch(p, sg);
    a_stage = npix * 32 > a_stage ? npix * 32 : a_stage;
    if (sg.ntaps > CONV_MAXTAPS || sg.ntaps > CONV_BT * (CONV_BS - 1) || npix > 0x3FFF) return cudaErrorInvalidValue;
    for (int t = 0; t < sg.ntaps; ++t) p.seg[s].aoff[t] = (sg.dh[t] + sg.ht) * pitch + sg.dw[t] + sg.hl;
  }
  p.a_stage = (a_stage + 255) & ~255;
  p.as = CONV_AS;
  p.bs = CONV_BS;
  auto rings_fit = [&](int as, int bs) {
    return (size_t)as * p.a_stage + (size_t)bs * CONV_B_SLOT + CONV_STAGING + 2048 <= (size_t)CONV_SMEM_MAX;
  };
  while (p.as < 6 && rings_fit(p.as + 1, p.bs)) ++p.as;
  while (p.bs < CONV_BS_MAX && rings_fit(p.as, p.bs + 1)) ++p.bs;
  while (p.as < CONV_AS_MAX && rings_fit(p.as + 1, p.bs)) ++p.as;
  if (conv_smem_bytes(p) > (size_t)CONV_SMEM_MAX) return cudaErrorInvalidValue;
  return cudaSuccess;
}

cudaError_t launch_conv_tc(const ConvParams& p_in, int num_sms, cudaStream_t stream) {
  ConvParams p = p_in;
  p.dbg = conv_dbg_env();
  if (cudaError_t e = plan_conv_tc(p, num_sms)) return e;
  ConvMaps maps{};
  if (p.tile2d) {
    for (int s = 0; s < p.nseg; ++s) {
      const ConvSeg& sg = p.seg[s];
      cudaError_t e = encode_pf8_map(&maps.src[s], sg.src + (long long)p.lead * 8, p, 1, p.Wp, p.PL, 2 * sg.ksteps,
                                     sg.img_stride, p.tw + sg.hl + sg.hr, p.th + sg.ht + sg.hb, 2);
      if (e != cudaSuccess) return e;
    }
    const int bh = p.th, bplanes = p.tw == 16 ? 1 : 8;
    cudaError_t e;
    if (p.up2) {
      const Geom og = make_geom(p.N, 2 * p.H, 2 * p.W);
      e = encode_pf8_map(&maps.out, p.out + (long long)(og.lead + p.oy * og.Wp + p.ox) * 8, p, 2, 2 * og.Wp, og.PL,
                         p.cout / 8, (long long)(p.cout / 8) * og.PL * 8, 8, bh, bplanes);
    } else {
      e = encode_pf8_map(&maps.out, p.out + (long long)p.lead * 8, p, 1, p.Wp, p.PL, p.cout / 8,
                         (long long)(p.cout / 8) * p.PL * 8, 8, bh, bplanes);
    }
    if (e != cudaSuccess) return e;
  }
  const size_t smem = conv_smem_bytes(p);
  const int grid = p.total_work < num_sms ? p.total_work : num_sms;
  if (grid <= 0) return cudaSuccess;
  const bool square = p.tile2d && p.tw == 16;
  void (*kernel)(ConvParams, ConvMaps) = square ? conv_tc_kernel<true> : conv_tc_kernel<false>;
  static size_t attr[2] = {0, 0};
  if (smem > attr[square]) {
    cudaError_t e = cudaFuncSetAttribute(kernel, cudaFuncAttributeMaxDynamicSharedMemorySize, (int)smem);
    if (e != cudaSuccess) return e;
    attr[square] = smem;
  }
  cudaLaunchConfig_t cfg = {};
  cfg.gridDim = dim3((unsigned)grid);
  cfg.blockDim = dim3(CONV_THREADS);
  cfg.dynamicSmemBytes = smem;
  cfg.stream = stream;
  cudaLaunchAttribute at[1];
  at[0].id = cudaLaunchAttributeProgrammaticStreamSerialization;
  at[0].val.programmaticStreamSerializationAllowed = 1;
  cfg.attrs = at;
  cfg.numAttrs = 1;
  return cudaLaunchKernelEx(&cfg, kernel, p, maps);
}

__global__ void pack_identity_kernel(int channels, __nv_bfloat16* __restrict__ dst, long long nvec) {
  const long long id = (long long)blockIdx.x * blockDim.x + threadIdx.x;
  if (id >= nvec) return;
  const int r = (int)(id & 7), n8 = (int)((id >> 3) & 15), k8 = (int)((id >> 7) & 1);
  const long long rest = id >> 8;
  const int ksteps = channels / 16;
  const int ks = (int)(rest % ksteps), ntile = (int)(rest / ksteps);
  const int co = ntile * 128 + n8 * 8 + r;
  const int ci0 = ks * 16 + k8 * 8;
  uint32_t o[4];
#pragma unroll
  for (int e = 0; e < 4; ++e) o[e] = pack_bf16x2(co == ci0 + 2 * e ? 1.f : 0.f, co == ci0 + 2 * e + 1 ? 1.f : 0.f);
  reinterpret_cast<uint4*>(dst)[id] = make_uint4(o[0], o[1], o[2], o[3]);
}
cudaError_t launch_pack_identity(int channels, __nv_bfloat16* dst, cudaStream_t s) {
  const long long nvec = (long long)(channels / 128) * (channels / 16) * 256;
  pack_identity_kernel<<<(unsigned)((nvec + 255) / 256), 256, 0, s>>>(channels, dst, nvec);
  return cudaGetLastError();
}

}
```

### audio_diffusion_b200/csrc/conv_tc.cuh

```cuda
#pragma once
#include "common.cuh"

namespace b200ad {

constexpr int CONV_NT = 128;
constexpr int CONV_TM = 128;
constexpr int CONV_MAXG = 2;
constexpr int CONV_MAXSEG = 4;
constexpr int CONV_MAXTAPS = 9;
constexpr int CONV_B_TAP = 16 * CONV_NT * 2;
constexpr int CONV_SMEM_MAX = 227 * 1024;

constexpr int CONV_BT = 3;
constexpr int CONV_B_SLOT = CONV_BT * CONV_B_TAP;
constexpr int CONV_AS_MAX = 8;
constexpr int CONV_AS = 3;
constexpr int CONV_BS = 5;
constexpr int CONV_BS_MAX = 10;

struct ConvSeg {
  const __nv_bfloat16* src;
  const __nv_bfloat16* wpack;
  long long img_stride;
  long long wtile_stride;
  int ksteps;
  int ntaps;
  int ht, hb, hl, hr;
  signed char dh[CONV_MAXTAPS];
  signed char dw[CONV_MAXTAPS];
  int aoff[CONV_MAXTAPS];
  const float2* ss;
  int ss_stride;
  int silu;
};

struct ConvGnFin {
  const stat_t* stats[2];
  int C[2];
  const float* gamma;
  const float* beta;
  float2* ss;
  unsigned* counter;
  int groups, HW;
  float eps;
};

struct ConvParams {
  ConvSeg seg[CONV_MAXSEG];
  int nseg;
  int N, H, W, Wp, lead, PL;
  int a_stage;
  int tile2d;
  int tw, th;
  int tiles_y;
  int groups_per_img;
  int ntiles_n;
  int total_work;
  int pack;
  int as, bs;
  int cout;
  __nv_bfloat16* out;
  const float* bias;
  const float* temb;
  int temb_stride;
  stat_t* stats;
  int up2, oy, ox;
  ConvGnFin fin;
  int dbg;
};

cudaError_t plan_conv_tc(ConvParams& p, int num_sms);
int conv_dbg_env();
cudaError_t launch_conv_tc(const ConvParams& p, int num_sms, cudaStream_t stream);

cudaError_t launch_pack_identity(int channels, __nv_bfloat16* dst, cudaStream_t s);

}
```

### audio_diffusion_b200/csrc/net.cuh

```cuda
#pragma once
#include <cstdarg>
#include <cstdio>
#include <cstdlib>
#include <cstring>
#include <functional>
#include <map>
#include <string>
#include <vector>

#include "../../include/b200ad.h"
#include "taps.cuh"

namespace b200ad {

int set_err(const char* fmt, ...);
#define CK(call)                                                                  \
  do {                                                                            \
    cudaError_t e__ = (call);                                                     \
    if (e__ != cudaSuccess) return set_err("%s: %s", #call, cudaGetErrorString(e__)); \
  } while (0)

struct Param {
  std::string name;
  std::vector<int64_t> shape;
};

struct Act {
  __nv_bfloat16* p = nullptr;
  int C = 0, H = 0, W = 0;
  stat_t* stats = nullptr;
  size_t off = 0;
};

enum OpKind { OP_TEMB = 0, OP_CONV_IN = 1, OP_GN = 2, OP_CONV = 3, OP_PARITY = 5, OP_ATTN = 6, OP_CONV_OUT = 7,
              OP_ATTN1 = 8 , OP_VAE_SAMPLE = 9, OP_MIX1X1 = 10,
              OP_LN = 11 , OP_GEGLU = 12, OP_MHA = 13 ,
              OP_XVEC = 14 ,
              OP_GNAPPLY = 15 ,
              OP_PACK_T , OP_DGRAD, OP_WGRAD, OP_GN_BWD, OP_CHANSUM,
              OP_REDUCE_N, OP_SCATTER, OP_PF8ADD, OP_ATTN_BWD, OP_UNFOLD, OP_SCALAR_WGRAD, OP_CONV_IN_BWD, OP_FLIP, OP_SUMADD,
              OP_LIN_IN, OP_LIN_W, OP_SILU_BWD, OP_SILU_FWD, OP_MEMSET, OP_LN_BWD, OP_GEGLU_BWD, OP_XVEC_BWD, OP_MHA_BWD,
              OP_ATTN1_BWD, OP_QUANT_BWD, OP_LATENT_IN_BWD, OP_NKINDS };
static const char* const op_names[] = {
    "temb", "conv_in", "gn_finalize", "conv_tc", "", "parity_split", "attention", "conv_out", "attention_1head", "vae_sample",
    "mix1x1", "layernorm", "geglu", "mha", "cross_attn_vec", "gn_apply", "pack_transposed", "conv_tc(dgrad)", "wgrad_tc",
    "gn_bwd", "chan_sum", "reduce_n", "scatter", "pf8_add", "attention_bwd", "unfold_up2", "scalar_wgrad", "conv_in(dgrad)",
    "flip", "sum_add", "lin_in", "lin_w", "silu_bwd", "silu_fwd", "memset", "layernorm_bwd", "geglu_bwd",
    "cross_attn_vec_bwd", "mha_bwd", "attention_1head_bwd", "quant_conv_bwd", "latent_in_bwd"};
static_assert(sizeof(op_names) / sizeof(op_names[0]) == OP_NKINDS, "one name per OpKind");

struct RunArgs {
  const float* in = nullptr;
  const float* t = nullptr;
  const float* noise = nullptr;
  float* out = nullptr;
  float* moments = nullptr;
  float* x_out = nullptr;
  const b200ad_step_coef* coef = nullptr;
  const b200ad_step_coef* coef_dev = nullptr;
  const float* g_eps = nullptr;
  const float* g_mom = nullptr;
  float* g_z = nullptr;
};

using OpFn = std::function<cudaError_t(const RunArgs&, cudaStream_t)>;
struct Op {
  OpKind kind;
  int launches = 1;
  ConvParams conv;
  OpFn run;
};

struct Bump {
  uint8_t* base = nullptr;
  size_t off = 0;
  void* take(size_t bytes) {
    off = (off + 255) & ~(size_t)255;
    void* r = base ? base + off : nullptr;
    off += bytes;
    return r;
  }
};
static size_t take_off(Bump& b, size_t bytes) {
  b.take(0);
  const size_t o = (b.off + 255) & ~(size_t)255;
  b.take(bytes);
  return o;
}
static Act take_act(Bump& b, int N, int C, int H, int W) {
  Act a;
  a.C = C; a.H = H; a.W = W;
  a.off = take_off(b, (size_t)N * (C / 8) * make_geom(N, H, W).PL * 16);
  a.p = b.base ? (__nv_bfloat16*)(b.base + a.off) : nullptr;
  return a;
}

struct PackJob {
  int w_param;
  int cout, cin_total, KH, KW, cin_off, ksteps;
  PackTaps taps;
  size_t off;
  int cout_real = -1;
};

struct FusedBias {
  enum Kind { SUM2,
              QKV,
              PAD128 }
    kind;
  int p[3];
  size_t off;
};

enum BlockKind {
  BK_UNET_HEAD,
  BK_CONV_IN,
  BK_LATENT_IN,
  BK_RESNET,
  BK_ATTN,
  BK_TRANSFORMER,
  BK_DOWN,
  BK_DOWN_ASYM,
  BK_UP,
  BK_CONV_OUT,
  BK_LATENT_OUT,
};
struct Block {
  BlockKind kind;
  std::string name;
  int in = -1, skip = -1;
  int cin = 0, cskip = 0, cout = 0;
  int temb = 0;
  int cross = 0;
  std::string pool;
  size_t conv1[2] = {}, conv2 = 0, shortcut[2] = {};
  size_t qkv = 0, out = 0;
  size_t proj_in = 0, ff1 = 0, ff2 = 0, proj_out = 0;
  size_t seg[4] = {};
  size_t ident = 0;
  size_t bias = 0;
  int temb_row = -1;
};
static Block& add_block(std::vector<Block>& bl, BlockKind kind, const std::string& name, int cin, int cout,
                        const char* pool) {
  Block b;
  b.kind = kind; b.name = name; b.in = (int)bl.size() - 1; b.cin = cin; b.cout = cout; b.pool = pool;
  bl.push_back(b);
  return bl.back();
}

struct OpList {
  std::vector<Op> ops;
  stat_t* stats = nullptr;
  size_t stats_bytes = 0;
};
struct Plan {
  std::vector<OpList> lists;
  std::map<std::string, Act> taps;
  float* temb_act = nullptr;
  float* temb_proj = nullptr;
  int* temb_lead = nullptr;
  float* temb_emb = nullptr;
  float* temb_u1 = nullptr;
  float* temb_u2 = nullptr;
  float* zq = nullptr;
  std::map<std::string, float*> lse;
  std::map<std::string, float*> probs;
  float* z_in = nullptr;
  size_t ws_bytes = 0;
};

struct Backward;

struct NetBase {
  int norm_groups = 32;
  float norm_eps = 1e-5f;
  std::vector<Param> params;
  std::map<std::string, int> pidx;
  std::vector<const float*> pptr;
  std::vector<PackJob> jobs;
  std::map<int, size_t> ident_off;
  std::vector<FusedBias> fused;
  size_t packed_bytes = 0;
  size_t off_wcat = 0, off_bcat = 0;
  int temb_rows = 0;
  uint8_t* packed = nullptr;
  int N = 0, H = 0, W = 0;
  uint8_t* ws = nullptr;
  size_t ws_bytes = 0;
  Plan plan;
  bool training = false;
  int num_sms = 132;
  const float* enc = nullptr;
  int enc_S = 0;
  int last_launches = 0;
  PackBatch pack_batch;
  int nparts = 1;
  Backward* bwd[2] = {};
};
void release_backward(NetBase* h);

static PackItem make_pack_item(const NetBase* h, const PackJob& j, uint8_t* arena) {
  PackItem it;
  memset(&it, 0, sizeof(it));
  it.w = h->pptr[j.w_param];
  it.dst = (__nv_bfloat16*)(arena + j.off);
  it.cout = j.cout; it.cin_total = j.cin_total; it.KH = j.KH; it.KW = j.KW; it.cin_off = j.cin_off; it.ksteps = j.ksteps;
  it.cout_real = j.cout_real < 0 ? j.cout : j.cout_real;
  it.taps = j.taps;
  it.nvec = (long long)(j.cout / 128) * j.ksteps * j.taps.ntaps * 256;
  return it;
}

static int check_net_config(int num_blocks, const int* ch, int out_channels, int groups) {
  if (num_blocks < 1 || num_blocks > B200AD_MAX_BLOCKS) return set_err("num_blocks out of range");
  for (int i = 0; i < num_blocks; ++i)
    if (ch[i] % 128) return set_err("block_out_channels must be multiples of 128");
  if (out_channels > 4) return set_err("out_channels > 4 not implemented");
  if (groups < 1 || groups > 64) return set_err("norm_num_groups must be in 1..64");
  for (int i = 0; i < num_blocks; ++i)
    if (ch[i] % groups || (ch[i] / groups) % 4)
      return set_err("channels per GroupNorm group must be a multiple of 4 for every block");
  return 0;
}

static std::string S(const char* fmt, ...) {
  char buf[256];
  va_list ap;
  va_start(ap, fmt);
  vsnprintf(buf, sizeof(buf), fmt, ap);
  va_end(ap);
  return buf;
}

static int param_shape(const NetBase* h, int i, int64_t* dims) {
  const auto& s = h->params[i].shape;
  for (size_t k = 0; k < s.size(); ++k) dims[k] = s[k];
  return (int)s.size();
}
static void add_param(NetBase* h, const std::string& name, std::vector<int64_t> shape) {
  h->pidx[name] = (int)h->params.size();
  h->params.push_back({name, std::move(shape)});
}
static void p_conv(NetBase* h, const std::string& n, int cin, int cout, int k) {
  add_param(h, n + ".weight", {cout, cin, k, k});
  add_param(h, n + ".bias", {cout});
}
static void p_lin(NetBase* h, const std::string& n, int cin, int cout) {
  add_param(h, n + ".weight", {cout, cin});
  add_param(h, n + ".bias", {cout});
}
static void p_gn(NetBase* h, const std::string& n, int c) {
  add_param(h, n + ".weight", {c});
  add_param(h, n + ".bias", {c});
}
static void p_resnet(NetBase* h, const std::string& n, int cin, int cout, int temb) {
  p_gn(h, n + ".norm1", cin);
  p_conv(h, n + ".conv1", cin, cout, 3);
  if (temb) p_lin(h, n + ".time_emb_proj", temb, cout);
  p_gn(h, n + ".norm2", cout);
  p_conv(h, n + ".conv2", cout, cout, 3);
  if (cin != cout) p_conv(h, n + ".conv_shortcut", cin, cout, 1);
}
static void p_attn(NetBase* h, const std::string& n, int c) {
  p_gn(h, n + ".group_norm", c);
  p_lin(h, n + ".to_q", c, c);
  p_lin(h, n + ".to_k", c, c);
  p_lin(h, n + ".to_v", c, c);
  p_lin(h, n + ".to_out.0", c, c);
}
static void p_transformer(NetBase* h, const std::string& n, int c, int X) {
  p_gn(h, n + ".norm", c);
  p_conv(h, n + ".proj_in", c, c, 1);
  const std::string b = n + ".transformer_blocks.0";
  p_gn(h, b + ".norm1", c);
  add_param(h, b + ".attn1.to_q.weight", {c, c});
  add_param(h, b + ".attn1.to_k.weight", {c, c});
  add_param(h, b + ".attn1.to_v.weight", {c, c});
  p_lin(h, b + ".attn1.to_out.0", c, c);
  p_gn(h, b + ".norm2", c);
  add_param(h, b + ".attn2.to_q.weight", {c, c});
  add_param(h, b + ".attn2.to_k.weight", {c, X});
  add_param(h, b + ".attn2.to_v.weight", {c, X});
  p_lin(h, b + ".attn2.to_out.0", c, c);
  p_gn(h, b + ".norm3", c);
  p_lin(h, b + ".ff.net.0.proj", c, 8 * c);
  p_lin(h, b + ".ff.net.2", 4 * c, c);
  p_conv(h, n + ".proj_out", c, c, 1);
}
static void p_block(NetBase* h, const Block& k) {
  const std::string& n = k.name;
  switch (k.kind) {
    case BK_UNET_HEAD:
      p_conv(h, n + "conv_in", k.cin, k.cout, 3);
      p_lin(h, "time_embedding.linear_1", k.cout, k.temb);
      p_lin(h, "time_embedding.linear_2", k.temb, k.temb);
      break;
    case BK_CONV_IN: p_conv(h, n + "conv_in", k.cin, k.cout, 3); break;
    case BK_LATENT_IN:
      p_conv(h, "post_quant_conv", k.cin, k.cin, 1);
      p_conv(h, n + "conv_in", k.cin, k.cout, 3);
      break;
    case BK_RESNET: p_resnet(h, n, k.cin + k.cskip, k.cout, k.temb); break;
    case BK_ATTN: p_attn(h, n, k.cout); break;
    case BK_TRANSFORMER: p_transformer(h, n, k.cout, k.cross); break;
    case BK_DOWN: case BK_DOWN_ASYM: case BK_UP: p_conv(h, n, k.cout, k.cout, 3); break;
    case BK_CONV_OUT:
      p_gn(h, n + "conv_norm_out", k.cin);
      p_conv(h, n + "conv_out", k.cin, k.cout, 3);
      break;
    case BK_LATENT_OUT:
      p_gn(h, n + "conv_norm_out", k.cin);
      p_conv(h, n + "conv_out", k.cin, k.cout, 3);
      p_conv(h, "quant_conv", k.cout, k.cout, 1);
      break;
  }
}

static size_t add_job(NetBase* h, Bump& b, const std::string& wname, int cout, int cin_total, int K, int cin_off,
                      int cin_cnt, const TapSet& taps, int cout_real = -1) {
  PackJob j;
  j.w_param = h->pidx.at(wname);
  j.cout = cout; j.cin_total = cin_total; j.KH = K; j.KW = K; j.cin_off = cin_off; j.ksteps = cin_cnt / 16;
  j.taps = taps.pack;
  j.cout_real = cout_real;
  j.off = take_off(b, (size_t)(cout / 128) * j.ksteps * taps.pack.ntaps * CONV_B_TAP);
  h->jobs.push_back(j);
  return j.off;
}
static size_t add_ident(NetBase* h, Bump& b, int ch) {
  auto it = h->ident_off.find(ch);
  if (it == h->ident_off.end()) it = h->ident_off.emplace(ch, take_off(b, (size_t)(ch / 128) * (ch / 16) * CONV_B_TAP)).first;
  return it->second;
}
static size_t add_bias(NetBase* h, Bump& b, FusedBias::Kind kind, size_t floats, const std::string& p0,
                       const std::string& p1 = "", const std::string& p2 = "") {
  FusedBias f;
  f.kind = kind;
  f.p[0] = h->pidx.at(p0);
  f.p[1] = p1.empty() ? -1 : h->pidx.at(p1);
  f.p[2] = p2.empty() ? -1 : h->pidx.at(p2);
  f.off = take_off(b, floats * 4);
  h->fused.push_back(f);
  return f.off;
}
static TapSet down_taps(const Block& k, int a, int b) {
  return k.kind == BK_DOWN ? taps_parity(a, b) : taps_parity_asym(a, b);
}
static void layout_resnet(NetBase* h, Bump& b, Block& k) {
  const std::string& n = k.name;
  const int ca = k.cin, cb = k.cskip, co = k.cout, cin = ca + cb;
  k.conv1[0] = add_job(h, b, n + ".conv1.weight", co, cin, 3, 0, ca, taps_conv(3));
  if (cb) k.conv1[1] = add_job(h, b, n + ".conv1.weight", co, cin, 3, ca, cb, taps_conv(3));
  k.conv2 = add_job(h, b, n + ".conv2.weight", co, co, 3, 0, co, taps_conv(3));
  if (cin == co) {
    k.ident = add_ident(h, b, co);
  } else {
    k.shortcut[0] = add_job(h, b, n + ".conv_shortcut.weight", co, cin, 1, 0, ca, taps_conv(1));
    if (cb) k.shortcut[1] = add_job(h, b, n + ".conv_shortcut.weight", co, cin, 1, ca, cb, taps_conv(1));
    k.bias = add_bias(h, b, FusedBias::SUM2, co, n + ".conv2.bias", n + ".conv_shortcut.bias");
  }
  if (k.temb) {
    k.temb_row = h->temb_rows;
    h->temb_rows += co;
  }
}
static void layout_attn(NetBase* h, Bump& b, Block& k) {
  const std::string& n = k.name;
  const int ch = k.cout;
  k.qkv = add_job(h, b, n + ".to_q.weight", ch, ch, 1, 0, ch, taps_conv(1));
  add_job(h, b, n + ".to_k.weight", ch, ch, 1, 0, ch, taps_conv(1));
  add_job(h, b, n + ".to_v.weight", ch, ch, 1, 0, ch, taps_conv(1));
  k.out = add_job(h, b, n + ".to_out.0.weight", ch, ch, 1, 0, ch, taps_conv(1));
  k.bias = add_bias(h, b, FusedBias::QKV, (size_t)3 * ch, n + ".to_q.bias", n + ".to_k.bias", n + ".to_v.bias");
  k.ident = add_ident(h, b, ch);
}
static void layout_transformer(NetBase* h, Bump& b, Block& k) {
  const std::string& n = k.name;
  const std::string t = n + ".transformer_blocks.0";
  const int c = k.cout;
  k.proj_in = add_job(h, b, n + ".proj_in.weight", c, c, 1, 0, c, taps_conv(1));
  k.qkv = add_job(h, b, t + ".attn1.to_q.weight", c, c, 1, 0, c, taps_conv(1));
  add_job(h, b, t + ".attn1.to_k.weight", c, c, 1, 0, c, taps_conv(1));
  add_job(h, b, t + ".attn1.to_v.weight", c, c, 1, 0, c, taps_conv(1));
  k.out = add_job(h, b, t + ".attn1.to_out.0.weight", c, c, 1, 0, c, taps_conv(1));
  k.ff1 = add_job(h, b, t + ".ff.net.0.proj.weight", 8 * c, c, 1, 0, c, taps_conv(1));
  k.ff2 = add_job(h, b, t + ".ff.net.2.weight", c, 4 * c, 1, 0, 4 * c, taps_conv(1));
  k.proj_out = add_job(h, b, n + ".proj_out.weight", c, c, 1, 0, c, taps_conv(1));
  k.ident = add_ident(h, b, c);
}
static void layout_block(NetBase* h, Bump& b, Block& k) {
  switch (k.kind) {
    case BK_RESNET: layout_resnet(h, b, k); break;
    case BK_ATTN: layout_attn(h, b, k); break;
    case BK_TRANSFORMER: layout_transformer(h, b, k); break;
    case BK_DOWN: case BK_DOWN_ASYM:
      for (int a = 0; a < 2; ++a)
        for (int c = 0; c < 2; ++c)
          k.seg[a * 2 + c] = add_job(h, b, k.name + ".weight", k.cout, k.cout, 3, 0, k.cout, down_taps(k, a, c));
      break;
    case BK_UP:
      for (int a = 0; a < 2; ++a)
        for (int c = 0; c < 2; ++c)
          k.seg[a * 2 + c] = add_job(h, b, k.name + ".weight", k.cout, k.cout, 3, 0, k.cout, taps_up2(a, c));
      break;
    case BK_LATENT_OUT:
      k.seg[0] = add_job(h, b, k.name + "conv_out.weight", 128, k.cin, 3, 0, k.cin, taps_conv(3), k.cout);
      k.bias = add_bias(h, b, FusedBias::PAD128, 128, k.name + "conv_out.bias");
      break;
    default: break;
  }
}

static __global__ void add_vec_kernel(const float* a, const float* b, float* o, int n) {
  const int i = blockIdx.x * blockDim.x + threadIdx.x;
  if (i < n) o[i] = a[i] + (b ? b[i] : 0.f);
}

static int pack_common(NetBase* h, cudaStream_t st) {
  {
    std::vector<PackItem> items;
    items.reserve(h->jobs.size());
    for (const PackJob& j : h->jobs) items.push_back(make_pack_item(h, j, h->packed));
    CK(launch_pack_batch(h->pack_batch, items, st));
  }
  for (const auto& kv : h->ident_off) CK(launch_pack_identity(kv.first, (__nv_bfloat16*)(h->packed + kv.second), st));
  for (const FusedBias& f : h->fused) {
    float* dst = (float*)(h->packed + f.off);
    const int c = (int)h->params[f.p[0]].shape[0];
    const float* const* src = h->pptr.data();
    switch (f.kind) {
      case FusedBias::SUM2:
        add_vec_kernel<<<(c + 255) / 256, 256, 0, st>>>(src[f.p[0]], src[f.p[1]], dst, c);
        CK(cudaGetLastError());
        break;
      case FusedBias::QKV:
        for (int i = 0; i < 3; ++i) CK(cudaMemcpyAsync(dst + i * c, src[f.p[i]], c * 4, cudaMemcpyDeviceToDevice, st));
        break;
      case FusedBias::PAD128:
        CK(cudaMemsetAsync(dst, 0, 128 * 4, st));
        CK(cudaMemcpyAsync(dst, src[f.p[0]], c * 4, cudaMemcpyDeviceToDevice, st));
        break;
    }
  }
  return 0;
}

static ConvParams conv_geom(int N, const Act& out) {
  const Geom g = make_geom(N, out.H, out.W);
  ConvParams p{};
  p.N = N; p.H = out.H; p.W = out.W; p.Wp = g.Wp; p.lead = g.lead; p.PL = g.PL;
  p.cout = out.C;
  p.out = out.p;
  p.stats = out.stats;
  return p;
}
static GnApplyParams gn_params(const NetBase* h, int N, const Act& a, const Act* b, const std::string& norm,
                               __nv_bfloat16* dst, bool silu, float eps = -1.f) {
  GnApplyParams p{};
  p.src[0] = a.p; p.stats[0] = a.stats; p.C[0] = a.C;
  p.src[1] = b ? b->p : nullptr; p.stats[1] = b ? b->stats : nullptr; p.C[1] = b ? b->C : 0;
  p.gamma = h->pptr[h->pidx.at(norm + ".weight")]; p.beta = h->pptr[h->pidx.at(norm + ".bias")];
  p.dst = dst;
  p.N = N; p.H = a.H; p.W = a.W; p.groups = h->norm_groups; p.eps = eps < 0.f ? h->norm_eps : eps; p.silu = silu ? 1 : 0;
  return p;
}

struct Builder {
  const NetBase* h;
  Plan* built;
  Bump ws;
  Bump st;
  std::vector<Op>* ops;
  std::map<std::string, Act> pool;
  int N, H = 0, W = 0;
  int heads = 8;
  bool nopool = false;
  bool single_head = false;

  Act alloc(int C, int H, int W, bool stats) {
    Act a = take_act(ws, N, C, H, W);
    if (stats) a.stats = (stat_t*)st.take((size_t)N * (C / 4) * 2 * sizeof(stat_t));
    return a;
  }
  Act pooled(const std::string& tag, int C, int H, int W, bool stats) {
    const std::string key = S("%s:%d:%d:%d", tag.c_str(), C, H, W);
    if (nopool) return alloc(C, H, W, stats);
    auto it = pool.find(key);
    if (it == pool.end()) it = pool.emplace(key, alloc(C, H, W, false)).first;
    Act a = it->second;
    if (stats) a.stats = (stat_t*)st.take((size_t)N * (C / 4) * 2 * sizeof(stat_t));
    return a;
  }
  Act output(const Block& k, int C, int H, int W) {
    return k.pool.empty() ? alloc(C, H, W, true) : pooled(k.pool, C, H, W, true);
  }
  const float* P(const std::string& name) const { return h->pptr[h->pidx.at(name)]; }
  template <class T> const T* PK(size_t off) const { return h->packed ? (const T*)(h->packed + off) : nullptr; }

  void emit(OpKind kind, OpFn run, int launches = 1) { ops->push_back(Op{kind, launches, {}, std::move(run)}); }
  void conv(const ConvParams& p) {
    Op op{OP_CONV};
    op.conv = p;
    ops->push_back(op);
  }
  void seg(ConvSeg& s, const __nv_bfloat16* src, int C, int H, int W, size_t woff, const TapSet& t) {
    set_seg(s, src, C / 8, C, H, W, PK<__nv_bfloat16>(woff), t);
  }
  void seg(ConvSeg& s, const Act& a, size_t woff, const TapSet& t) { seg(s, a.p, a.C, a.H, a.W, woff, t); }

  float2* gn_attach(const Act& a, const Act* b, const std::string& norm, float2* ss = nullptr, float eps = -1.f) {
    const int Ct = a.C + (b ? b->C : 0);
    if (ops->empty() || ops->back().kind != OP_CONV || ops->back().conv.out != a.p || ops->back().conv.fin.ss ||
        (size_t)N * h->norm_groups * 2 * sizeof(float) > 32768)
      return nullptr;
    if (!ss) ss = (float2*)ws.take((size_t)N * Ct * sizeof(float2));
    ConvGnFin& f = ops->back().conv.fin;
    f.stats[0] = a.stats; f.C[0] = a.C;
    f.stats[1] = b ? b->stats : nullptr; f.C[1] = b ? b->C : 0;
    f.gamma = P(norm + ".weight"); f.beta = P(norm + ".bias");
    f.ss = ss;
    f.counter = (unsigned*)ws.take(sizeof(unsigned));
    f.groups = h->norm_groups; f.HW = a.H * a.W; f.eps = eps < 0.f ? h->norm_eps : eps;
    return ss;
  }

  float2* gn_finalize(const Act& a, const Act* b, const std::string& norm, float eps = -1.f) {
    const int Ct = a.C + (b ? b->C : 0);
    float2* ss = (float2*)ws.take((size_t)N * Ct * sizeof(float2));
    if (gn_attach(a, b, norm, ss, eps)) return ss;
    const GnApplyParams p = gn_params(h, N, a, b, norm, nullptr, false, eps);
    emit(OP_GN, [p, ss](const RunArgs&, cudaStream_t s) { return launch_gn_finalize(p, ss, s); });
    return ss;
  }
  static void seg_norm(ConvSeg& s, const float2* ss, int stride, bool silu) {
    s.ss = ss; s.ss_stride = stride; s.silu = silu ? 1 : 0;
  }

  Act conv_in(const Block& k, const float* src) {
    Act x = output(k, k.cout, H, W);
    emit(OP_CONV_IN, [src, w = P(k.name + "conv_in.weight"), b = P(k.name + "conv_in.bias"), N = N, cin = k.cin, H = H,
                      W = W, x](const RunArgs& a, cudaStream_t s) {
      return launch_conv_in(src ? src : a.in, w, b, N, cin, H, W, x.C, x.p, x.stats, s);
    });
    built->taps[k.name + "conv_in"] = x;
    return x;
  }

  Act unet_head(const Block& k) {
    built->temb_act = (float*)ws.take((size_t)N * k.temb * 4);
    built->temb_proj = (float*)ws.take((size_t)N * h->temb_rows * 4);
    built->temb_lead = (int*)ws.take((size_t)N * 4);
    if (h->training) {
      built->temb_emb = (float*)ws.take((size_t)N * k.cout * 4);
      built->temb_u1 = (float*)ws.take((size_t)N * k.temb * 4);
      built->temb_u2 = (float*)ws.take((size_t)N * k.temb * 4);
    }
    const Plan& pl = *built;
    emit(OP_TEMB, [h = h, dim0 = k.cout, act = pl.temb_act, proj = pl.temb_proj, emb = pl.temb_emb, u1 = pl.temb_u1,
                   u2 = pl.temb_u2, lead = h->training ? nullptr : pl.temb_lead](const RunArgs& a, cudaStream_t s) {
      auto P = [h](const char* name) { return h->pptr[h->pidx.at(name)]; };
      return launch_temb(a.t, h->N, dim0, P("time_embedding.linear_1.weight"), P("time_embedding.linear_1.bias"),
                         P("time_embedding.linear_2.weight"), P("time_embedding.linear_2.bias"), act,
                         (const float*)(h->packed + h->off_wcat), (const float*)(h->packed + h->off_bcat), h->temb_rows,
                         proj, s, emb, u1, u2, lead);
    }, 2);
    return conv_in(k, nullptr);
  }

  Act latent_in(const Block& k) {
    float* zq = built->zq = (float*)ws.take((size_t)N * k.cin * H * W * 4);
    float* z_in = h->training ? built->z_in = (float*)ws.take((size_t)N * k.cin * H * W * 4) : nullptr;
    emit(OP_MIX1X1, [zq, z_in, w = P("post_quant_conv.weight"), b = P("post_quant_conv.bias"), N = N, L = k.cin, H = H,
                     W = W](const RunArgs& a, cudaStream_t s) {
      if (z_in) {
        const cudaError_t e = cudaMemcpyAsync(z_in, a.in, (size_t)N * L * H * W * 4, cudaMemcpyDeviceToDevice, s);
        if (e != cudaSuccess) return e;
      }
      return launch_mix1x1(a.in, w, b, zq, N, L, H * W, s);
    });
    return conv_in(k, zq);
  }

  Act resnet(const Block& k, const Act& a, const Act* b) {
    const std::string& n = k.name;
    const int cin = a.C + (b ? b->C : 0), cout = k.cout;
    const int H = a.H, W = a.W;
    const float2* ss1 = gn_finalize(a, b, n + ".norm1");
    Act h1 = pooled("h1", cout, H, W, true);
    {
      ConvParams p = conv_geom(N, h1);
      p.nseg = 1;
      seg(p.seg[0], a, k.conv1[0], taps_conv(3));
      seg_norm(p.seg[0], ss1, cin, true);
      if (b) {
        seg(p.seg[1], *b, k.conv1[1], taps_conv(3));
        seg_norm(p.seg[1], ss1 + a.C, cin, true);
        p.nseg = 2;
      }
      p.bias = P(n + ".conv1.bias");
      if (k.temb_row >= 0) {
        p.temb = built->temb_proj + k.temb_row;
        p.temb_stride = h->temb_rows;
      }
      conv(p);
    }
    const float2* ss2 = gn_finalize(h1, nullptr, n + ".norm2");
    Act out = output(k, cout, H, W);
    {
      ConvParams p = conv_geom(N, out);
      p.nseg = 1;
      seg(p.seg[0], h1, k.conv2, taps_conv(3));
      seg_norm(p.seg[0], ss2, cout, true);
      if (cin != cout) {
        seg(p.seg[1], a, k.shortcut[0], taps_conv(1));
        p.nseg = 2;
        if (b) {
          seg(p.seg[2], *b, k.shortcut[1], taps_conv(1));
          p.nseg = 3;
        }
        p.bias = PK<float>(k.bias);
      } else {
        seg(p.seg[1], a, k.ident, taps_conv(1));
        p.nseg = 2;
        p.bias = P(n + ".conv2.bias");
      }
      conv(p);
    }
    built->taps[n + ".h1"] = h1;
    built->taps[n] = out;
    return out;
  }

  void linear(const Act& out, const Act& src, size_t woff, const float* bias, const float2* ss = nullptr,
              const Act* residual = nullptr, size_t ident = 0, const float* vec = nullptr, int vec_stride = 0) {
    ConvParams p = conv_geom(N, out);
    p.nseg = 1;
    seg(p.seg[0], src, woff, taps_conv(1));
    if (ss) seg_norm(p.seg[0], ss, src.C, false);
    if (residual) {
      seg(p.seg[1], *residual, ident, taps_conv(1));
      p.nseg = 2;
    }
    p.bias = bias;
    p.temb = vec; p.temb_stride = vec_stride;
    conv(p);
  }

  Act transformer(const Block& k, const Act& x) {
    const std::string& n = k.name;
    const int C = x.C, H = x.H, W = x.W;
    const std::string t = n + ".transformer_blocks.0";
    const float2* ssx = gn_finalize(x, nullptr, n + ".norm", 1e-6f);
    float* vec = (float*)ws.take((size_t)N * C * sizeof(float));
    emit(OP_XVEC, [h = h, wv = P(t + ".attn2.to_v.weight"), wo = P(t + ".attn2.to_out.0.weight"),
                   bo = P(t + ".attn2.to_out.0.bias"), vec, N = N, C, X = k.cross](const RunArgs&, cudaStream_t s) {
      return launch_cross_attn_vec(h->enc, wv, wo, bo, vec, N, C, X, s);
    });
    Act h0 = pooled("tf_h0", C, H, W, false);
    linear(h0, x, k.proj_in, P(n + ".proj_in.bias"), ssx);
    Act n1 = pooled("tf_ln", C, H, W, false);
    auto layer_norm = [&](const Act& src, const Act& dst, const std::string& nm) {
      emit(OP_LN, [x = src.p, y = dst.p, g = P(nm + ".weight"), b = P(nm + ".bias"), N = N, C, H, W](const RunArgs&,
                                                                                                      cudaStream_t s) {
        return launch_layernorm_pf8(x, y, g, b, N, C, H, W, 1e-5f, s);
      });
    };
    layer_norm(h0, n1, t + ".norm1");
    Act qkv = pooled("tf_qkv", 3 * C, H, W, false);
    linear(qkv, n1, k.qkv, nullptr);
    Act ao = pooled("tf_ao", C, H, W, false);
    float* lse = h->training ? built->lse[n] = (float*)ws.take((size_t)N * heads * H * W * sizeof(float)) : nullptr;
    emit(OP_MHA, [q = qkv.p, o = ao.p, N = N, C, heads = heads, H, W, lse](const RunArgs&, cudaStream_t s) {
      return launch_mha_flash(q, o, N, C, heads, H, W, s, lse);
    });
    Act h2 = pooled("tf_h2", C, H, W, false);
    linear(h2, ao, k.out, P(t + ".attn1.to_out.0.bias"), nullptr, &h0, k.ident, vec, C);
    Act n3 = pooled("tf_ln", C, H, W, false);
    layer_norm(h2, n3, t + ".norm3");
    Act ff1 = pooled("tf_ff1", 8 * C, H, W, false);
    linear(ff1, n3, k.ff1, P(t + ".ff.net.0.proj.bias"));
    Act gg = pooled("tf_gg", 4 * C, H, W, false);
    emit(OP_GEGLU, [x = ff1.p, y = gg.p, N = N, C, H, W](const RunArgs&, cudaStream_t s) {
      return launch_geglu_pf8(x, y, N, 4 * C, H, W, s);
    });
    Act h3 = pooled("tf_h0", C, H, W, false);
    linear(h3, gg, k.ff2, P(t + ".ff.net.2.bias"), nullptr, &h2, k.ident);
    Act out = output(k, C, H, W);
    linear(out, h3, k.proj_out, P(n + ".proj_out.bias"), nullptr, &x, k.ident);
    built->taps[n + ".attn2"] = h2;
    built->taps[n] = out;
    if (h->training) {
      built->taps[n + ".h0"] = h0;
      built->taps[n + ".n1"] = n1;
      built->taps[n + ".qkv"] = qkv;
      built->taps[n + ".ao"] = ao;
      built->taps[n + ".n3"] = n3;
      built->taps[n + ".ff1"] = ff1;
      built->taps[n + ".gg"] = gg;
      built->taps[n + ".h3"] = h3;
    }
    return out;
  }

  Act down2(const Block& k, const Act& x) {
    const int C = x.C, Ho = x.H / 2, Wo = x.W / 2;
    const Geom go = make_geom(N, Ho, Wo);
    const size_t tsz = (size_t)N * (C / 8) * go.PL * 8;
    Act par = pooled("parity", 4 * C, Ho, Wo, false);
    built->taps[k.name + ".parity"] = par;
    emit(OP_PARITY, [x, par = par.p, N = N](const RunArgs&, cudaStream_t s) {
      return launch_parity_split(x.p, par, N, x.C, x.H, x.W, s);
    });
    Act y = output(k, C, Ho, Wo);
    ConvParams p = conv_geom(N, y);
    p.nseg = 4;
    for (int a = 0; a < 2; ++a)
      for (int b = 0; b < 2; ++b)
        seg(p.seg[a * 2 + b], par.p + (size_t)(a * 2 + b) * tsz, C, Ho, Wo, k.seg[a * 2 + b], down_taps(k, a, b));
    p.bias = P(k.name + ".bias");
    conv(p);
    built->taps[k.name] = y;
    return y;
  }

  Act up2(const Block& k, const Act& x) {
    const int C = x.C, hh = x.H, ww = x.W;
    Act y = output(k, C, hh * 2, ww * 2);
    for (int pa = 0; pa < 2; ++pa)
      for (int pb = 0; pb < 2; ++pb) {
        Act lo = y;
        lo.H = hh; lo.W = ww;
        ConvParams p = conv_geom(N, lo);
        p.up2 = 1; p.oy = pa; p.ox = pb;
        p.nseg = 1;
        seg(p.seg[0], x, k.seg[pa * 2 + pb], taps_up2(pa, pb));
        p.bias = P(k.name + ".bias");
        conv(p);
      }
    built->taps[k.name] = y;
    return y;
  }

  Act attention(const Block& k, const Act& x) {
    const std::string& n = k.name;
    const int C = x.C, H = x.H, W = x.W;
    Act xn = pooled("attn_xn", C, H, W, false);
    const GnApplyParams g = gn_params(h, N, x, nullptr, n + ".group_norm", xn.p, false);
    emit(OP_GNAPPLY, [g](const RunArgs&, cudaStream_t s) { return launch_gn_apply(g, s); });
    Act qkv = pooled("qkv", 3 * C, H, W, false);
    linear(qkv, xn, k.qkv, PK<float>(k.bias));
    Act ao = pooled("attn_o", C, H, W, false);
    if (single_head) {
      float* scores = (float*)ws.take((size_t)N * H * W * H * W * sizeof(float));
      if (h->training) built->probs[n] = scores;
      emit(OP_ATTN1, [q = qkv.p, o = ao.p, scores, N = N, C, H, W](const RunArgs&, cudaStream_t s) {
        return launch_attention_1head(q, o, scores, N, C, H, W, s);
      }, 3);
    } else {
      emit(OP_ATTN, [q = qkv.p, o = ao.p, N = N, C, H, W](const RunArgs&, cudaStream_t s) {
        return launch_attention(q, o, N, C, H, W, s);
      });
    }
    Act out = output(k, C, H, W);
    linear(out, ao, k.out, P(n + ".to_out.0.bias"), nullptr, &x, k.ident);
    built->taps[n + ".qkv"] = qkv;
    built->taps[n + ".ao"] = ao;
    built->taps[n] = out;
    return out;
  }

  Act conv_out(const Block& k, const Act& x) {
    const std::string& n = k.name;
    ConvOutParams p{};
    p.src = x.p; p.stats = x.stats;
    p.ss = gn_attach(x, nullptr, n + "conv_norm_out");
    p.gamma = P(n + "conv_norm_out.weight"); p.beta = P(n + "conv_norm_out.bias");
    p.w = P(n + "conv_out.weight"); p.b = P(n + "conv_out.bias");
    p.N = N; p.C = x.C; p.H = x.H; p.W = x.W; p.cout = k.cout; p.groups = h->norm_groups; p.eps = h->norm_eps;
    emit(OP_CONV_OUT, [p](const RunArgs& a, cudaStream_t s) {
      ConvOutParams q = p;
      q.eps_out = a.out;
      q.x = a.in; q.z = a.noise; q.x_out = a.x_out;
      static_assert(sizeof(b200ad_step_coef) == sizeof(StepCoef), "step-coefficient layouts differ");
      q.coef_dev = reinterpret_cast<const StepCoef*>(a.coef_dev);
      if (a.coef) memcpy(&q.coef, a.coef, sizeof(StepCoef));
      return launch_conv_out(q, s);
    });
    built->taps[n + "pre_out"] = x;
    return x;
  }

  Act latent_out(const Block& k, const Act& x) {
    const std::string& n = k.name;
    Act eo = pooled("enc_out", 128, x.H, x.W, false);
    {
      const float2* ss = gn_finalize(x, nullptr, n + "conv_norm_out");
      ConvParams p = conv_geom(N, eo);
      p.nseg = 1;
      seg(p.seg[0], x, k.seg[0], taps_conv(3));
      seg_norm(p.seg[0], ss, x.C, true);
      p.bias = PK<float>(k.bias);
      conv(p);
    }
    built->taps[n + "conv_out"] = eo;
    emit(OP_VAE_SAMPLE, [eo = eo.p, w = P("quant_conv.weight"), b = P("quant_conv.bias"), N = N, L = k.cout / 2, H = x.H,
                         W = x.W](const RunArgs& a, cudaStream_t s) {
      return launch_vae_sample(eo, w, b, a.noise, a.out, a.moments, N, 128, L, H, W, s);
    });
    return eo;
  }

  void run(const std::vector<Block>& blocks) {
    std::vector<Act> outs(blocks.size());
    for (size_t i = 0; i < blocks.size(); ++i) {
      const Block& k = blocks[i];
      const Act* x = k.in >= 0 ? &outs[k.in] : nullptr;
      const Act* skip = k.skip >= 0 ? &outs[k.skip] : nullptr;
      switch (k.kind) {
        case BK_UNET_HEAD: outs[i] = unet_head(k); break;
        case BK_CONV_IN: outs[i] = conv_in(k, nullptr); break;
        case BK_LATENT_IN: outs[i] = latent_in(k); break;
        case BK_RESNET: outs[i] = resnet(k, *x, skip); break;
        case BK_ATTN: outs[i] = attention(k, *x); break;
        case BK_TRANSFORMER: outs[i] = transformer(k, *x); break;
        case BK_DOWN: case BK_DOWN_ASYM: outs[i] = down2(k, *x); break;
        case BK_UP: outs[i] = up2(k, *x); break;
        case BK_CONV_OUT: outs[i] = conv_out(k, *x); break;
        case BK_LATENT_OUT: outs[i] = latent_out(k, *x); break;
      }
    }
  }
};

static bool debug_nopool() {
  const char* e = getenv("B200AD_DEBUG_NOPOOL");
  return e && e[0] == '1';
}

template <class Net>
static int bind_workspace(Net* h, Plan (*build)(const Net*, uint8_t*, int, int, int), void* workspace, size_t bytes, int N,
                          int H, int W, cudaStream_t st) {
  if (!h->packed) return set_err("set_params must be called before bind_workspace");
  const int down = 1 << (h->cfg.num_blocks - 1);
  if (H % down || W % down) return set_err("H and W must be multiples of %d", down);
  const size_t need = build(h, nullptr, N, H, W).ws_bytes;
  if (bytes < need) return set_err("workspace too small: %zu < %zu", bytes, need);
  CK(cudaMemsetAsync(workspace, 0, need, st));
  h->plan = build(h, (uint8_t*)workspace, N, H, W);
  h->N = N; h->H = H; h->W = W;
  h->ws = (uint8_t*)workspace; h->ws_bytes = need;
  int dev = 0;
  CK(cudaGetDevice(&dev));
  CK(cudaDeviceGetAttribute(&h->num_sms, cudaDevAttrMultiProcessorCount, dev));
  return 0;
}

static int set_training(NetBase* h, int on) {
  if (!h) return set_err("null handle");
  if (h->training != (on != 0)) {
    h->training = on != 0;
    h->plan.lists.clear();
  }
  return 0;
}

struct OpEvents {
  std::vector<cudaEvent_t> ev;
  ~OpEvents() {
    for (cudaEvent_t e : ev)
      if (e) cudaEventDestroy(e);
  }
  int ms(size_t i, float* out) const {
    CK(cudaEventElapsedTime(out, ev[i], ev[i + 1]));
    return 0;
  }
};

static int run_ops(const NetBase* h, const OpList& l, const RunArgs& a, cudaStream_t st, int* launches,
                   OpEvents* timing = nullptr) {
  if (l.stats_bytes) CK(cudaMemsetAsync(l.stats, 0, l.stats_bytes, st));
  if (timing) {
    timing->ev.assign(l.ops.size() + 1, nullptr);
    for (cudaEvent_t& e : timing->ev) CK(cudaEventCreate(&e));
    CK(cudaEventRecord(timing->ev[0], st));
  }
  int n = 0;
  for (size_t i = 0; i < l.ops.size(); ++i) {
    const Op& op = l.ops[i];
    const cudaError_t e = op.run ? op.run(a, st) : launch_conv_tc(op.conv, h->num_sms, st);
    if (e != cudaSuccess) return set_err("%s: %s", op_names[op.kind], cudaGetErrorString(e));
    if (timing) CK(cudaEventRecord(timing->ev[i + 1], st));
    n += op.launches;
  }
  *launches = n;
  return 0;
}

static int debug_tensor(const NetBase* h, const char* name, float* dst, int* dims, cudaStream_t st) {
  auto it = h->plan.taps.find(name);
  if (it == h->plan.taps.end()) return set_err("unknown tap '%s'", name);
  const Act& a = it->second;
  if (dims) { dims[0] = a.C; dims[1] = a.H; dims[2] = a.W; }
  if (dst) CK(launch_pf8_to_nchw(a.p, dst, h->N, a.C, a.H, a.W, st));
  return a.C;
}

}
```

### audio_diffusion_b200/csrc/unet.cu

```cuda
#include "unet.cuh"

namespace b200ad {

thread_local char g_err[512] = "";
int set_err(const char* fmt, ...) {
  va_list ap;
  va_start(ap, fmt);
  vsnprintf(g_err, sizeof(g_err), fmt, ap);
  va_end(ap);
  return -1;
}

}

using namespace b200ad;


namespace b200ad {

static std::vector<Block> unet_blocks(const b200ad_unet_config& c) {
  const int nb = c.num_blocks, D = c.block_out_channels[0] * 4, X = c.cross_attention_dim;
  const int* boc = c.block_out_channels;
  std::vector<Block> bl;
  add_block(bl, BK_UNET_HEAD, "", c.in_channels, boc[0], "").temb = D;
  std::vector<int> skips{0};
  auto attn = [&](const std::string& n, bool self, bool cross, int ch, const char* pool) {
    if (self || cross) add_block(bl, cross ? BK_TRANSFORMER : BK_ATTN, n, ch, ch, pool).cross = cross ? X : 0;
  };
  for (int i = 0; i < nb; ++i) {
    for (int j = 0; j < c.layers_per_block; ++j) {
      const bool att = c.down_attn[i] || c.down_cross[i];
      add_block(bl, BK_RESNET, S("down_blocks.%d.resnets.%d", i, j), bl.back().cout, boc[i], att ? "res_tmp" : "").temb = D;
      attn(S("down_blocks.%d.attentions.%d", i, j), c.down_attn[i], c.down_cross[i], boc[i], "");
      skips.push_back((int)bl.size() - 1);
    }
    if (i != nb - 1) {
      add_block(bl, BK_DOWN, S("down_blocks.%d.downsamplers.0.conv", i), boc[i], boc[i], "");
      skips.push_back((int)bl.size() - 1);
    }
  }
  const int mid = boc[nb - 1];
  add_block(bl, BK_RESNET, "mid_block.resnets.0", mid, mid, "res_tmp").temb = D;
  attn("mid_block.attentions.0", !X, X != 0, mid, "up_a");
  add_block(bl, BK_RESNET, "mid_block.resnets.1", mid, mid, "up_b").temb = D;
  int flip = 0;
  for (int i = 0; i < nb; ++i) {
    const int out_c = boc[nb - 1 - i];
    for (int j = 0; j < c.layers_per_block + 1; ++j) {
      const bool att = c.up_attn[i] || c.up_cross[i];
      const int sk = skips.back();
      skips.pop_back();
      Block& r = add_block(bl, BK_RESNET, S("up_blocks.%d.resnets.%d", i, j), bl.back().cout, out_c,
                           att ? "res_tmp" : (flip++ & 1) ? "up_b" : "up_a");
      r.skip = sk;
      r.cskip = bl[sk].cout;
      r.temb = D;
      if (att) attn(S("up_blocks.%d.attentions.%d", i, j), c.up_attn[i], c.up_cross[i], out_c, (flip++ & 1) ? "up_b" : "up_a");
    }
    if (i != nb - 1) add_block(bl, BK_UP, S("up_blocks.%d.upsamplers.0.conv", i), out_c, out_c, "up_conv");
  }
  add_block(bl, BK_CONV_OUT, "", boc[0], c.out_channels, "");
  return bl;
}

}

extern "C" const char* b200ad_last_error(void) { return g_err; }
extern "C" int b200ad_version(void) { return 1; }

extern "C" int b200ad_unet_create(const b200ad_unet_config* cfg, b200ad_unet** out) {
  if (!cfg || !out) return set_err("null argument");
  if (check_net_config(cfg->num_blocks, cfg->block_out_channels, cfg->out_channels, cfg->norm_num_groups)) return -1;
  if (cfg->attention_head_dim != 8) return set_err("only attention_head_dim == 8 is implemented");
  if (cfg->cross_attention_dim < 0 || cfg->cross_attention_dim > 4096) return set_err("cross_attention_dim out of range");
  for (int i = 0; i < cfg->num_blocks; ++i) {
    if ((cfg->down_cross[i] || cfg->up_cross[i]) && !cfg->cross_attention_dim) return set_err("cross-attention blocks need cross_attention_dim");
    if ((cfg->down_cross[i] && cfg->down_attn[i]) || (cfg->up_cross[i] && cfg->up_attn[i])) return set_err("a block is either Attn or CrossAttn");
    const int d = cfg->block_out_channels[i] / 8;
    if ((cfg->down_cross[i] || cfg->up_cross[i]) && d != 16 && d != 32 && d != 64) return set_err("cross-attention blocks need channels / 8 in {16, 32, 64}");
  }
  b200ad_unet* h = new b200ad_unet();
  h->cfg = *cfg;
  h->norm_groups = cfg->norm_num_groups;
  h->norm_eps = cfg->norm_eps;
  h->blocks = unet_blocks(*cfg);
  for (const Block& k : h->blocks) p_block(h, k);
  Bump b;
  for (Block& k : h->blocks) layout_block(h, b, k);
  const int D = cfg->block_out_channels[0] * 4;
  h->off_wcat = take_off(b, (size_t)h->temb_rows * D * 4);
  h->off_bcat = take_off(b, (size_t)h->temb_rows * 4);
  h->packed_bytes = (b.off + 255) & ~(size_t)255;
  h->pptr.assign(h->params.size(), nullptr);
  *out = h;
  return 0;
}
extern "C" void b200ad_unet_destroy(b200ad_unet* h) {
  if (!h) return;
  release_backward(h);
  delete h;
}
extern "C" int b200ad_unet_num_params(const b200ad_unet* h) { return (int)h->params.size(); }
extern "C" const char* b200ad_unet_param_name(const b200ad_unet* h, int i) { return h->params[i].name.c_str(); }
extern "C" int b200ad_unet_param_shape(const b200ad_unet* h, int i, int64_t* dims) { return param_shape(h, i, dims); }
extern "C" size_t b200ad_unet_packed_bytes(const b200ad_unet* h) { return h->packed_bytes; }

extern "C" int b200ad_unet_set_params(b200ad_unet* h, const float* const* params, void* packed, size_t packed_bytes,
                                      void* stream) {
  if (packed_bytes < h->packed_bytes) return set_err("packed buffer too small: %zu < %zu", packed_bytes, h->packed_bytes);
  cudaStream_t st = (cudaStream_t)stream;
  for (size_t i = 0; i < h->params.size(); ++i) h->pptr[i] = params[i];
  h->packed = (uint8_t*)packed;
  if (pack_common(h, st)) return -1;
  const int D = h->cfg.block_out_channels[0] * 4;
  for (const Block& k : h->blocks) {
    if (k.temb_row < 0) continue;
    CK(cudaMemcpyAsync(h->packed + h->off_wcat + (size_t)k.temb_row * D * 4,
                       h->pptr[h->pidx.at(k.name + ".time_emb_proj.weight")], (size_t)k.cout * D * 4,
                       cudaMemcpyDeviceToDevice, st));
    CK(cudaMemcpyAsync(h->packed + h->off_bcat + (size_t)k.temb_row * 4,
                       h->pptr[h->pidx.at(k.name + ".time_emb_proj.bias")], (size_t)k.cout * 4, cudaMemcpyDeviceToDevice, st));
  }
  return 0;
}

namespace b200ad {

static Plan build_plan(const b200ad_unet* h, uint8_t* ws_base, int N, int H, int W) {
  Plan pl;
  pl.lists.resize(1);
  OpList& l = pl.lists[0];
  Builder B;
  B.h = h; B.built = &pl; B.ops = &l.ops;
  B.N = N; B.H = H; B.W = W;
  B.heads = h->cfg.attention_head_dim;
  B.nopool = debug_nopool() || h->training;
  B.ws.base = ws_base;
  for (int pass = 0; pass < 2; ++pass) {
    l.ops.clear();
    B.pool.clear();
    pl.taps.clear();
    B.st.base = pass == 0 ? nullptr : ws_base;
    B.st.off = 0;
    B.ws.off = pass == 0 ? 0 : ((l.stats_bytes + 255) & ~(size_t)255);
    B.run(h->blocks);
    if (pass == 0) l.stats_bytes = B.st.off;
  }
  l.stats = (stat_t*)ws_base;
  pl.ws_bytes = (B.ws.off + 255) & ~(size_t)255;
  return pl;
}

}

extern "C" size_t b200ad_unet_workspace_bytes(const b200ad_unet* h, int N, int H, int W) {
  return build_plan(h, nullptr, N, H, W).ws_bytes;
}

extern "C" int b200ad_unet_bind_workspace(b200ad_unet* h, void* workspace, size_t bytes, int N, int H, int W, void* stream) {
  return bind_workspace(h, build_plan, workspace, bytes, N, H, W, (cudaStream_t)stream);
}

static int run_plan(b200ad_unet* h, const RunArgs& a, cudaStream_t st, OpEvents* timing = nullptr) {
  if (h->plan.lists.empty()) return set_err("bind_workspace must be called before forward");
  if (h->cfg.cross_attention_dim) {
    if (!h->enc) return set_err("conditional U-Net: call b200ad_unet_set_encoding before forward");
    if (h->enc_S != 1) return set_err("conditional U-Net: encoder sequence length %d (only 1 is implemented)", h->enc_S);
  }
  return run_ops(h, h->plan.lists[0], a, st, &h->last_launches, timing);
}

extern "C" int b200ad_unet_profile_step(b200ad_unet* h, const float* x, const float* t, const float* z,
                                        const b200ad_step_coef* coef, float* x_out, float* op_ms, int* op_kind,
                                        double* op_flops, int max_ops, void* stream) {
  if (h->plan.lists.empty()) return set_err("bind_workspace must be called before profile_step");
  cudaStream_t st = (cudaStream_t)stream;
  const std::vector<Op>& ops = h->plan.lists[0].ops;
  const int nops = (int)ops.size();
  if (nops > max_ops) return set_err("profile_step: %d ops > max_ops %d", nops, max_ops);
  RunArgs a;
  a.in = x; a.t = t; a.noise = z; a.coef = coef; a.x_out = x_out;
  OpEvents ev;
  if (run_plan(h, a, st, &ev)) return -1;
  CK(cudaStreamSynchronize(st));
  for (int i = 0; i < nops; ++i) {
    if (ev.ms(i, &op_ms[i])) return -1;
    op_kind[i] = (int)ops[i].kind;
    double fl = 0;
    if (ops[i].kind == OP_CONV) {
      const ConvParams& p = ops[i].conv;
      double k = 0;
      for (int s = 0; s < p.nseg; ++s) {
        bool ident = false;
        for (const auto& kv : h->ident_off)
          if ((const uint8_t*)p.seg[s].wpack == h->packed + kv.second) ident = true;
        if (!ident) k += (double)(p.up2 ? 9 : p.seg[s].ntaps) * p.seg[s].ksteps * 16;
      }
      fl = 2.0 * p.N * p.H * p.W * p.cout * k;
    }
    op_flops[i] = fl;
  }
  return nops;
}

extern "C" int b200ad_unet_conv_plan(const b200ad_unet* h, int N, int H, int W, int num_sms, int* rows, int max_rows) {
  const Plan pl = build_plan(h, nullptr, N, H, W);
  const int dbg = conv_dbg_env();
  int n = 0;
  for (const Op& op : pl.lists[0].ops) {
    if (op.kind != OP_CONV) continue;
    if (n >= max_rows) return set_err("conv_plan: more than %d conv launches", max_rows);
    ConvParams p = op.conv;
    p.dbg = dbg;
    if (plan_conv_tc(p, num_sms) != cudaSuccess) return set_err("conv_plan: launch %d cannot be planned", n);
    const int row[B200AD_CONV_PLAN_COLS] = {p.H, p.W, p.seg[0].ksteps * 16, p.cout, p.nseg, p.up2,
                                             p.pack, p.tw, p.th, p.total_work, p.as, p.bs};
    for (int c = 0; c < B200AD_CONV_PLAN_COLS; ++c) rows[n * B200AD_CONV_PLAN_COLS + c] = row[c];
    ++n;
  }
  return n;
}

extern "C" int b200ad_unet_set_encoding(b200ad_unet* h, const float* enc, int S) {
  if (!h->cfg.cross_attention_dim) return set_err("set_encoding: this U-Net is unconditional");
  if (S < 1) return set_err("set_encoding: empty encoder sequence");
  h->enc = enc;
  h->enc_S = S;
  return 0;
}

extern "C" int b200ad_unet_forward(b200ad_unet* h, const float* x, const float* t, float* eps_out, void* stream) {
  RunArgs a;
  a.in = x; a.t = t; a.out = eps_out;
  return run_plan(h, a, (cudaStream_t)stream);
}
extern "C" int b200ad_unet_forward_step(b200ad_unet* h, const float* x, const float* t, const float* z,
                                        const b200ad_step_coef* coef, float* x_out, float* eps_out, void* stream) {
  if (!coef || !x_out) return set_err("coef and x_out are required");
  RunArgs a;
  a.in = x; a.t = t; a.noise = z; a.coef = coef; a.x_out = x_out; a.out = eps_out;
  return run_plan(h, a, (cudaStream_t)stream);
}
__global__ void step_scalars_kernel(b200ad_step_coef coef, float t, b200ad_step_coef* coef_dev, float* t_dev, int n) {
  const int i = blockIdx.x * blockDim.x + threadIdx.x;
  if (i == 0) *coef_dev = coef;
  if (i < n) t_dev[i] = t;
}
extern "C" int b200ad_step_scalars_upload(const b200ad_step_coef* coef, float t, b200ad_step_coef* coef_dev, float* t_dev, int n,
                                          void* stream) {
  if (!coef || !coef_dev || !t_dev || n < 1) return set_err("step_scalars_upload: bad arguments");
  step_scalars_kernel<<<(n + 255) / 256, 256, 0, (cudaStream_t)stream>>>(*coef, t, coef_dev, t_dev, n);
  CK(cudaGetLastError());
  return 0;
}
extern "C" int b200ad_unet_forward_step_dev(b200ad_unet* h, const float* x, const float* t, const float* z,
                                            const b200ad_step_coef* coef_dev, float* x_out, void* stream) {
  if (!coef_dev || !x_out) return set_err("coef_dev and x_out are required");
  RunArgs a;
  a.in = x; a.t = t; a.noise = z; a.coef_dev = coef_dev; a.x_out = x_out;
  return run_plan(h, a, (cudaStream_t)stream);
}
extern "C" int b200ad_unet_last_launch_count(const b200ad_unet* h) { return h->last_launches; }

extern "C" int b200ad_unet_debug_tensor(b200ad_unet* h, const char* name, float* dst, int* dims, void* stream) {
  return debug_tensor(h, name, dst, dims, (cudaStream_t)stream);
}
```

### include/b200ad.h

```cpp
#ifndef B200AD_H
#define B200AD_H
#include <stddef.h>
#include <stdint.h>

#ifdef __cplusplus
extern "C" {
#endif

#define B200AD_MAX_BLOCKS 8

const char* b200ad_last_error(void);
int b200ad_version(void);

typedef struct {
  int in_channels, out_channels;
  int layers_per_block;
  int num_blocks;
  int block_out_channels[B200AD_MAX_BLOCKS];
  int down_attn[B200AD_MAX_BLOCKS];
  int up_attn[B200AD_MAX_BLOCKS];
  int norm_num_groups;
  float norm_eps;
  int attention_head_dim;
  int cross_attention_dim;
  int down_cross[B200AD_MAX_BLOCKS];
  int up_cross[B200AD_MAX_BLOCKS];
} b200ad_unet_config;

typedef struct b200ad_unet b200ad_unet;

int b200ad_unet_create(const b200ad_unet_config* cfg, b200ad_unet** out);
void b200ad_unet_destroy(b200ad_unet* h);

int b200ad_unet_num_params(const b200ad_unet* h);
const char* b200ad_unet_param_name(const b200ad_unet* h, int i);
int b200ad_unet_param_shape(const b200ad_unet* h, int i, int64_t* dims);

size_t b200ad_unet_packed_bytes(const b200ad_unet* h);
size_t b200ad_unet_workspace_bytes(const b200ad_unet* h, int N, int H, int W);

int b200ad_unet_set_params(b200ad_unet* h, const float* const* params, void* packed, size_t packed_bytes, void* stream);

int b200ad_unet_bind_workspace(b200ad_unet* h, void* workspace, size_t bytes, int N, int H, int W, void* stream);

int b200ad_unet_forward(b200ad_unet* h, const float* x, const float* t, float* eps_out, void* stream);

int b200ad_unet_set_encoding(b200ad_unet* h, const float* enc, int S);

typedef struct {
  float sqrt_1m_at, inv_sqrt_at, clip, c_x0, c_xt, c_eps, c_z;
  int do_clip;
} b200ad_step_coef;

int b200ad_unet_forward_step(b200ad_unet* h, const float* x, const float* t, const float* z,
                             const b200ad_step_coef* coef, float* x_out, float* eps_out, void* stream);

int b200ad_unet_forward_step_dev(b200ad_unet* h, const float* x, const float* t, const float* z,
                                 const b200ad_step_coef* coef_dev, float* x_out, void* stream);
int b200ad_step_scalars_upload(const b200ad_step_coef* coef, float t, b200ad_step_coef* coef_dev, float* t_dev, int n,
                               void* stream);

int b200ad_unet_debug_tensor(b200ad_unet* h, const char* name, float* dst, int* dims, void* stream);

int b200ad_unet_profile_step(b200ad_unet* h, const float* x, const float* t, const float* z,
                             const b200ad_step_coef* coef, float* x_out, float* op_ms, int* op_kind,
                             double* op_flops, int max_ops, void* stream);

int b200ad_unet_last_launch_count(const b200ad_unet* h);

#define B200AD_CONV_PLAN_COLS 12
int b200ad_unet_conv_plan(const b200ad_unet* h, int N, int H, int W, int num_sms, int* rows, int max_rows);

int b200ad_unet_set_training(b200ad_unet* h, int on);
size_t b200ad_unet_grad_floats(b200ad_unet* h);
size_t b200ad_unet_grad_offset(b200ad_unet* h, int i);
size_t b200ad_unet_backward_bytes(b200ad_unet* h);
int b200ad_unet_bind_backward(b200ad_unet* h, void* arena, size_t bytes, float* grads, void* stream);
int b200ad_unet_backward(b200ad_unet* h, const float* x, const float* g_eps, int accumulate, void* stream);
int b200ad_unet_backward_launch_count(const b200ad_unet* h);
int b200ad_unet_debug_grad(b200ad_unet* h, const char* name, int skip, float* dst, int* dims, void* stream);

typedef struct {
  int in_channels, out_channels;
  int latent_channels;
  int layers_per_block;
  int num_blocks;
  int block_out_channels[B200AD_MAX_BLOCKS];
  int norm_num_groups;
  float norm_eps;
} b200ad_vae_config;

typedef struct b200ad_vae b200ad_vae;

int b200ad_vae_create(const b200ad_vae_config* cfg, b200ad_vae** out);
void b200ad_vae_destroy(b200ad_vae* h);
int b200ad_vae_num_params(const b200ad_vae* h);
const char* b200ad_vae_param_name(const b200ad_vae* h, int i);
int b200ad_vae_param_shape(const b200ad_vae* h, int i, int64_t* dims);
size_t b200ad_vae_packed_bytes(const b200ad_vae* h);
size_t b200ad_vae_workspace_bytes(const b200ad_vae* h, int N, int H, int W);
int b200ad_vae_set_params(b200ad_vae* h, const float* const* params, void* packed, size_t packed_bytes, void* stream);
int b200ad_vae_bind_workspace(b200ad_vae* h, void* workspace, size_t bytes, int N, int H, int W, void* stream);

int b200ad_vae_encode(b200ad_vae* h, const float* x, const float* noise, float* z, float* moments, void* stream);
int b200ad_vae_decode(b200ad_vae* h, const float* z, float* x_out, void* stream);
int b200ad_vae_debug_tensor(b200ad_vae* h, const char* name, float* dst, int* dims, void* stream);
int b200ad_vae_last_launch_count(const b200ad_vae* h);

int b200ad_vae_set_training(b200ad_vae* h, int on);
size_t b200ad_vae_grad_floats(b200ad_vae* h);
size_t b200ad_vae_grad_offset(b200ad_vae* h, int i);
size_t b200ad_vae_backward_bytes(b200ad_vae* h);
int b200ad_vae_bind_backward(b200ad_vae* h, void* arena, size_t bytes, float* grads, void* stream);
int b200ad_vae_decoder_backward(b200ad_vae* h, const float* g_x, float* g_z_out, int accumulate, void* stream);
int b200ad_vae_encoder_backward(b200ad_vae* h, const float* x, const float* g_moments, int accumulate, void* stream);
int b200ad_vae_backward_launch_count(const b200ad_vae* h);
int b200ad_vae_debug_grad(b200ad_vae* h, const char* name, int skip, float* dst, int* dims, void* stream);

typedef struct {
  float lr;
  float beta1, beta2;
  float eps;
  float weight_decay;
  float max_grad_norm;
  float ema_decay;
  int step;
} b200ad_optim_hparams;
typedef struct b200ad_optim b200ad_optim;
int b200ad_optim_create(int n_tensors, const int64_t* sizes, float* const* params, float* const* exp_avg,
                        float* const* exp_avg_sq, float* const* ema, b200ad_optim** out);
void b200ad_optim_destroy(b200ad_optim* h);
int b200ad_optim_step(b200ad_optim* h, const float* const* grads, const b200ad_optim_hparams* hp, float* grad_norm_out,
                      void* stream);
int b200ad_mse_loss_grad(const float* pred, const float* target, size_t n, float* loss_out, float* grad_out,
                         double* scratch, void* stream);

size_t b200ad_conv2d_scratch_bytes(int N, int cin, int cout, int H, int W, int K, int stride);
int b200ad_conv2d(const float* x, const float* w, const float* bias, const float* temb, const float* residual,
                  float* y, float* stats_out, int N, int cin, int cout, int H, int W, int K, int stride,
                  void* scratch, size_t scratch_bytes, void* stream);
int b200ad_gn_conv2d(const float* x, const float* gamma, const float* beta, int groups, float eps, int silu,
                     const float* w, const float* bias, float* y, int N, int cin, int cout, int H, int W, int K,
                     void* scratch, size_t scratch_bytes, void* stream);
int b200ad_conv2d_dgrad(const float* gy, const float* w, float* gx, int N, int cin, int cout, int H, int W, int K,
                        void* scratch, size_t scratch_bytes, void* stream);
size_t b200ad_conv2d_wgrad_scratch_bytes(int N, int cin, int cout, int H, int W);
int b200ad_conv2d_wgrad(const float* gy, const float* a, float* dw, int N, int cin, int cout, int H, int W, int K,
                        void* scratch, size_t scratch_bytes, void* stream);
size_t b200ad_mha_scratch_bytes(int N, int C, int heads, int H, int W);
int b200ad_mha_forward_backward(const float* q, const float* k, const float* v, const float* dout, float* out, float* dq,
                                float* dk, float* dv, int N, int C, int heads, int H, int W, void* scratch,
                                size_t scratch_bytes, void* stream);
int b200ad_group_norm(const float* x, const float* gamma, const float* beta, float* y, int N, int C, int H, int W,
                      int groups, float eps, int silu, void* scratch, size_t scratch_bytes, void* stream);

typedef struct {
  int x_res, y_res, sample_rate, n_fft, hop_length, top_db, n_iter;
} b200ad_mel_config;
size_t b200ad_mel_scratch_bytes(const b200ad_mel_config* cfg, int n);
int b200ad_mel_encode(const b200ad_mel_config* cfg, const float* mel_basis_t, const float* audio, uint8_t* images,
                      int n, void* scratch, size_t scratch_bytes, void* stream);
int b200ad_mel_encode_ref(const b200ad_mel_config* cfg, const float* mel_basis_t, const float* audio, uint8_t* images,
                          int n, const float* ref_values, float* mel_power_out, void* scratch, size_t scratch_bytes,
                          void* stream);
int b200ad_mel_decode(const b200ad_mel_config* cfg, const double* mel_pinv, const uint8_t* images, float* audio, int n,
                      uint64_t phase_seed, void* scratch, size_t scratch_bytes, void* stream);

int b200ad_sample_to_u8(const float* x, uint8_t* img, size_t n, void* stream);

#ifdef __cplusplus
}
#endif
#endif
```

Baseline: 0.9299.

## Add residual in conv epilogue instead of identity-weight GEMM segment

Residual connections were previously folded into the conv as an extra K-segment multiplied by a packed identity matrix, which costs tensor-core MMAs and extra weight traffic. The conv kernel now gets a RES template variant that TMA/bulk-loads the residual tile into shared memory during the main loop and adds it to the accumulators in the epilogue via ldmatrix.trans. This removes the identity weights and their packing, but adds an extra barrier, a shared-memory staging reuse and more template instantiations. It also adds a gn_conv2d_residual API entry and a query for which convs carry residuals.

```diff
diff --git a/audio_diffusion_b200/_lib.py b/audio_diffusion_b200/_lib.py
--- a/audio_diffusion_b200/_lib.py
+++ b/audio_diffusion_b200/_lib.py
@@ -65,6 +65,7 @@
     "b200ad_unet_debug_tensor": (_I, [_VP, C.c_char_p, _VP, C.POINTER(_I), _VP]),
     "b200ad_unet_last_launch_count": (_I, [_VP]),
     "b200ad_unet_conv_plan": (_I, [_VP, _I, _I, _I, _I, C.POINTER(_I), _I]),
+    "b200ad_unet_conv_residuals": (_I, [_VP, _I, _I, _I, C.POINTER(_I), _I]),
     "b200ad_unet_set_training": (_I, [_VP, _I]),
     "b200ad_unet_grad_floats": (_SZ, [_VP]),
     "b200ad_unet_grad_offset": (_SZ, [_VP, _I]),
@@ -106,6 +107,7 @@
     "b200ad_conv2d_wgrad_scratch_bytes": (_SZ, [_I] * 5),
     "b200ad_conv2d_wgrad": (_I, [_VP, _VP, _VP] + [_I] * 6 + [_VP, _SZ, _VP]),
     "b200ad_gn_conv2d": (_I, [_VP, _VP, _VP, _I, C.c_float, _I, _VP, _VP, _VP] + [_I] * 6 + [_VP, _SZ, _VP]),
+    "b200ad_gn_conv2d_residual": (_I, [_VP, _VP, _VP, _I, C.c_float, _I] + [_VP] * 6 + [_I] * 6 + [_VP, _SZ, _VP]),
     "b200ad_group_norm": (_I, [_VP] * 4 + [_I] * 5 + [C.c_float, _I, _VP, _SZ, _VP]),
     "b200ad_mha_scratch_bytes": (_SZ, [_I] * 5),
     "b200ad_mha_forward_backward": (_I, [_VP] * 8 + [_I] * 5 + [_VP, _SZ, _VP]),
diff --git a/audio_diffusion_b200/csrc/api.cu b/audio_diffusion_b200/csrc/api.cu
--- a/audio_diffusion_b200/csrc/api.cu
+++ b/audio_diffusion_b200/csrc/api.cu
@@ -19,7 +19,7 @@
 static size_t al(size_t x) { return (x + 255) & ~(size_t)255; }
 
 struct ConvScratch {
-  size_t x, par, res, out, wpack, ident, stats, instats, ss, total;
+  size_t x, par, res, out, wpack, stats, instats, ss, total;
 };
 static ConvScratch conv_scratch_layout(int N, int cin, int cout, int H, int W, int K, int stride) {
   ConvScratch s{};
@@ -32,7 +32,6 @@
   s.res = off; off = al(off + (size_t)N * (cout / 8) * go.PL * 16);
   s.out = off; off = al(off + (size_t)N * (cout / 8) * go.PL * 16);
   s.wpack = off; off = al(off + (size_t)(cout / 128) * (cin / 16) * (K * K > 16 ? K * K : 16) * CONV_B_TAP);
-  s.ident = off; off = al(off + (size_t)(cout / 128) * (cout / 16) * CONV_B_TAP);
   s.stats = off; off = al(off + (size_t)N * (cout / 4) * 2 * sizeof(stat_t));
   s.instats = off; off = al(off + (size_t)N * (cin / 4) * 2 * sizeof(stat_t));
   s.ss = off; off = al(off + (size_t)N * cin * sizeof(float2));
@@ -91,10 +90,8 @@
       s.ss = ss; s.ss_stride = cin; s.silu = gn_silu;
     }
     if (residual) {
-      __nv_bfloat16* ident = (__nv_bfloat16*)(sb + L.ident);
-      CK(launch_pack_identity(cout, ident, st));
-      set_seg(p.seg[1], rp, cout / 8, cout, Ho, Wo, ident, taps_conv(1));
-      p.nseg = 2;
+      p.res = rp;
+      p.res_img_stride = (long long)(cout / 8) * go.PL * 8;
     }
   } else if (stride == 2) {
     CK(launch_parity_split(xp, par, N, cin, H, W, st));
@@ -214,6 +211,15 @@
                      scratch, scratch_bytes, stream);
 }
 
+extern "C" int b200ad_gn_conv2d_residual(const float* x, const float* gamma, const float* beta, int groups, float eps,
+                                         int silu, const float* w, const float* bias, const float* temb,
+                                         const float* residual, float* y, float* stats_out, int N, int cin, int cout, int H,
+                                         int W, int K, void* scratch, size_t scratch_bytes, void* stream) {
+  if (!gamma || !beta) return set_err("gn_conv2d_residual: gamma and beta are required");
+  return conv2d_impl(x, w, bias, temb, residual, y, stats_out, N, cin, cout, H, W, K, 1, gamma, beta, groups, eps, silu,
+                     scratch, scratch_bytes, stream);
+}
+
 extern "C" int b200ad_group_norm(const float* x, const float* gamma, const float* beta, float* y, int N, int C, int H,
                                  int W, int groups, float eps, int silu, void* scratch, size_t scratch_bytes, void* stream) {
   if (C % 32) return set_err("group_norm: C %% 32 != 0");
diff --git a/audio_diffusion_b200/csrc/common.cuh b/audio_diffusion_b200/csrc/common.cuh
--- a/audio_diffusion_b200/csrc/common.cuh
+++ b/audio_diffusion_b200/csrc/common.cuh
@@ -274,6 +274,10 @@
   asm volatile("stmatrix.sync.aligned.m8n8.x4.trans.shared.b16 [%0], {%1, %2, %3, %4};"
                ::"r"(saddr), "r"(r0), "r"(r1), "r"(r2), "r"(r3) : "memory");
 }
+__device__ __forceinline__ void ldmatrix_x4_trans(uint32_t saddr, uint32_t& r0, uint32_t& r1, uint32_t& r2, uint32_t& r3) {
+  asm volatile("ldmatrix.sync.aligned.m8n8.x4.trans.shared.b16 {%0, %1, %2, %3}, [%4];"
+               : "=r"(r0), "=r"(r1), "=r"(r2), "=r"(r3) : "r"(saddr) : "memory");
+}
 
 __device__ __forceinline__ void mma_bf16_16x8x16(float (&c)[4], uint32_t a0, uint32_t a1, uint32_t a2, uint32_t a3, uint32_t b0,
                                                  uint32_t b1) {
diff --git a/audio_diffusion_b200/csrc/conv_tc.cu b/audio_diffusion_b200/csrc/conv_tc.cu
--- a/audio_diffusion_b200/csrc/conv_tc.cu
+++ b/audio_diffusion_b200/csrc/conv_tc.cu
@@ -10,6 +10,7 @@
 struct alignas(64) ConvMaps {
   CUtensorMap src[CONV_MAXSEG];
   CUtensorMap out;
+  CUtensorMap res;
 };
 
 __host__ __device__ __forceinline__ int window_pixels(const ConvParams& p, const ConvSeg& sg, int G) {
@@ -77,7 +78,7 @@
   return make_uint4(u[0], u[1], u[2], u[3]);
 }
 
-template <bool SQUARE>
+template <bool SQUARE, bool RES>
 __global__ void __launch_bounds__(CONV_THREADS, 1) conv_tc_kernel(const __grid_constant__ ConvParams p,
                                                                   const __grid_constant__ ConvMaps maps) {
   constexpr int ASM = CONV_AS_MAX, BSM = CONV_BS_MAX;
@@ -99,7 +100,8 @@
   const uint32_t bar_emptyA = smem_u32(bars + 2 * ASM);
   const uint32_t bar_fullB = smem_u32(bars + 3 * ASM);
   const uint32_t bar_emptyB = smem_u32(bars + 3 * ASM + BSM);
-  static_assert((3 * ASM + 2 * BSM) * 8 <= 1024, "barrier block overflows");
+  const uint32_t bar_res = smem_u32(bars + 3 * ASM + 2 * BSM);
+  static_assert((3 * ASM + 2 * BSM + 2) * 8 <= 1024, "barrier block overflows");
 
   if (warp == 1 && lane == 0) {
     for (int s = 0; s < AS; ++s) {
@@ -111,6 +113,8 @@
       mbar_init(bar_fullB + 8 * s, 1);
       mbar_init(bar_emptyB + 8 * s, 8);
     }
+    mbar_init(bar_res, 1);
+    mbar_init(bar_res + 8, 1);
     mbar_fence_init();
   }
   __syncthreads();
@@ -190,6 +194,8 @@
     const int hw_end = p.H * p.Wp;
     const bool do_stats = p.stats != nullptr;
     const bool issuer = tid < 8 * CONV_MAXG;
+    constexpr bool has_res = RES;
+    const uint32_t bar_res_w = bar_res + 8 * cw;
     float acc[CONV_MAXG * CONV_TM / 2];
     int sa = 0, sb = 0;
     uint32_t pa = 0, pb = 0;
@@ -197,6 +203,21 @@
       const WorkItem wi = decode_work(p, w);
 #pragma unroll
       for (int i = 0; i < CONV_MAXG * CONV_TM / 2; ++i) acc[i] = 0.f;
+      if (has_res && issuer) {
+        bulk_wait_read_all();
+        if (tid == 0) mbar_arrive_expect_tx(bar_res_w, (uint32_t)(wi.G * 8 * CONV_TM * 16));
+        const int g = tid >> 3, pl = tid & 7, plane = wi.ntile * 16 + cw * 8 + pl;
+        const uint32_t dst = stg_w + (uint32_t)(pl * CONV_SPLANE + g * CONV_TM * 16);
+        if (p.tile2d) {
+          if (SQUARE) tensor_g2s_4d(dst, &maps.res, 8 * (wi.c0 + 8 * g), wi.r0, plane, wi.n, bar_res_w);
+          else if (tid == 0) tensor_g2s_4d(stg_w, &maps.res, 8 * wi.c0, wi.r0, wi.ntile * 16 + cw * 8, wi.n, bar_res_w);
+        } else if (g < wi.G) {
+          const int n = p.pack ? wi.n + g : wi.n;
+          bulk_g2s(dst, p.res + (long long)n * p.res_img_stride + (long long)plane * p.PL * 8 +
+                            (long long)(p.lead + (p.pack ? 0 : wi.m0 + CONV_TM * g)) * 8,
+                   (uint32_t)CONV_TM * 16u, bar_res_w);
+        }
+      }
       int pend_b = -1, pend_a = -1;
       auto release = [&]() {
         __syncwarp();
@@ -243,7 +264,29 @@
 
       if (issuer) bulk_wait_read_all();
       named_bar_sync(1 + cw, 128);
+      if (has_res) mbar_wait(bar_res_w, ((w - blockIdx.x) / gridDim.x) & 1);
       if (!(p.dbg & 8)) {
+        if (has_res) {
+#pragma unroll
+          for (int g = 0; g < CONV_MAXG; ++g) {
+            if (g < wi.G) {
+#pragma unroll
+              for (int k = 0; k < CONV_TM / 16; ++k) {
+                uint32_t r[4];
+                ldmatrix_x4_trans(st_addr + (uint32_t)((g * CONV_TM + 16 * k) * 16), r[0], r[1], r[2], r[3]);
+#pragma unroll
+                for (int u = 0; u < 2; ++u)
+#pragma unroll
+                  for (int h = 0; h < 2; ++h) {
+                    const int j = g * (CONV_TM / 8) + 2 * k + u;
+                    const f32x2_t v = f2_from_bf16x2(r[2 * u + h]);
+                    acc[4 * j + 2 * h] = __fadd_rz(acc[4 * j + 2 * h], v.x);
+                    acc[4 * j + 2 * h + 1] = __fadd_rz(acc[4 * j + 2 * h + 1], v.y);
+                  }
+              }
+            }
+          }
+        }
         float ssum[2] = {0.f, 0.f}, ssq[2] = {0.f, 0.f};
 #pragma unroll
         for (int g = 0; g < CONV_MAXG; ++g) {
@@ -533,6 +576,7 @@
 
 cudaError_t plan_conv_tc(ConvParams& p, int num_sms) {
   if (p.nseg < 1 || p.nseg > CONV_MAXSEG) return cudaErrorInvalidValue;
+  if (p.res && p.up2) return cudaErrorInvalidValue;
   for (int s = 0; s < p.nseg; ++s) {
     ConvSeg& sg = p.seg[s];
     if (sg.ntaps > CONV_MAXTAPS || sg.ksteps < 1) return cudaErrorInvalidValue;
@@ -641,17 +685,24 @@
                          (long long)(p.cout / 8) * p.PL * 8, 8, bh, bplanes);
     }
     if (e != cudaSuccess) return e;
+    if (p.res) {
+      e = encode_pf8_map(&maps.res, p.res + (long long)p.lead * 8, p, 1, p.Wp, p.PL, p.cout / 8, p.res_img_stride, 8, bh,
+                         bplanes);
+      if (e != cudaSuccess) return e;
+    }
   }
   const size_t smem = conv_smem_bytes(p);
   const int grid = p.total_work < num_sms ? p.total_work : num_sms;
   if (grid <= 0) return cudaSuccess;
-  const bool square = p.tile2d && p.tw == 16;
-  void (*kernel)(ConvParams, ConvMaps) = square ? conv_tc_kernel<true> : conv_tc_kernel<false>;
-  static size_t attr[2] = {0, 0};
-  if (smem > attr[square]) {
+  const bool square = p.tile2d && p.tw == 16, res = p.res != nullptr;
+  void (*const kernels[2][2])(ConvParams, ConvMaps) = {{conv_tc_kernel<false, false>, conv_tc_kernel<false, true>},
+                                                       {conv_tc_kernel<true, false>, conv_tc_kernel<true, true>}};
+  void (*kernel)(ConvParams, ConvMaps) = kernels[square][res];
+  static size_t attr[2][2] = {};
+  if (smem > attr[square][res]) {
     cudaError_t e = cudaFuncSetAttribute(kernel, cudaFuncAttributeMaxDynamicSharedMemorySize, (int)smem);
     if (e != cudaSuccess) return e;
-    attr[square] = smem;
+    attr[square][res] = smem;
   }
   cudaLaunchConfig_t cfg = {};
   cfg.gridDim = dim3((unsigned)grid);
@@ -666,24 +717,4 @@
   return cudaLaunchKernelEx(&cfg, kernel, p, maps);
 }
 
-__global__ void pack_identity_kernel(int channels, __nv_bfloat16* __restrict__ dst, long long nvec) {
-  const long long id = (long long)blockIdx.x * blockDim.x + threadIdx.x;
-  if (id >= nvec) return;
-  const int r = (int)(id & 7), n8 = (int)((id >> 3) & 15), k8 = (int)((id >> 7) & 1);
-  const long long rest = id >> 8;
-  const int ksteps = channels / 16;
-  const int ks = (int)(rest % ksteps), ntile = (int)(rest / ksteps);
-  const int co = ntile * 128 + n8 * 8 + r;
-  const int ci0 = ks * 16 + k8 * 8;
-  uint32_t o[4];
-#pragma unroll
-  for (int e = 0; e < 4; ++e) o[e] = pack_bf16x2(co == ci0 + 2 * e ? 1.f : 0.f, co == ci0 + 2 * e + 1 ? 1.f : 0.f);
-  reinterpret_cast<uint4*>(dst)[id] = make_uint4(o[0], o[1], o[2], o[3]);
-}
-cudaError_t launch_pack_identity(int channels, __nv_bfloat16* dst, cudaStream_t s) {
-  const long long nvec = (long long)(channels / 128) * (channels / 16) * 256;
-  pack_identity_kernel<<<(unsigned)((nvec + 255) / 256), 256, 0, s>>>(channels, dst, nvec);
-  return cudaGetLastError();
-}
-
-}
+}
diff --git a/audio_diffusion_b200/csrc/conv_tc.cuh b/audio_diffusion_b200/csrc/conv_tc.cuh
--- a/audio_diffusion_b200/csrc/conv_tc.cuh
+++ b/audio_diffusion_b200/csrc/conv_tc.cuh
@@ -64,6 +64,8 @@
   const float* temb;
   int temb_stride;
   stat_t* stats;
+  const __nv_bfloat16* res;
+  long long res_img_stride;
   int up2, oy, ox;
   ConvGnFin fin;
   int dbg;
@@ -73,6 +75,4 @@
 int conv_dbg_env();
 cudaError_t launch_conv_tc(const ConvParams& p, int num_sms, cudaStream_t stream);
 
-cudaError_t launch_pack_identity(int channels, __nv_bfloat16* dst, cudaStream_t s);
-
 }
diff --git a/audio_diffusion_b200/csrc/net.cuh b/audio_diffusion_b200/csrc/net.cuh
--- a/audio_diffusion_b200/csrc/net.cuh
+++ b/audio_diffusion_b200/csrc/net.cuh
@@ -137,7 +137,6 @@
   size_t qkv = 0, out = 0;
   size_t proj_in = 0, ff1 = 0, ff2 = 0, proj_out = 0;
   size_t seg[4] = {};
-  size_t ident = 0;
   size_t bias = 0;
   int temb_row = -1;
 };
@@ -179,7 +178,6 @@
   std::map<std::string, int> pidx;
   std::vector<const float*> pptr;
   std::vector<PackJob> jobs;
-  std::map<int, size_t> ident_off;
   std::vector<FusedBias> fused;
   size_t packed_bytes = 0;
   size_t off_wcat = 0, off_bcat = 0;
@@ -328,11 +326,6 @@
   h->jobs.push_back(j);
   return j.off;
 }
-static size_t add_ident(NetBase* h, Bump& b, int ch) {
-  auto it = h->ident_off.find(ch);
-  if (it == h->ident_off.end()) it = h->ident_off.emplace(ch, take_off(b, (size_t)(ch / 128) * (ch / 16) * CONV_B_TAP)).first;
-  return it->second;
-}
 static size_t add_bias(NetBase* h, Bump& b, FusedBias::Kind kind, size_t floats, const std::string& p0,
                        const std::string& p1 = "", const std::string& p2 = "") {
   FusedBias f;
@@ -353,9 +346,7 @@
   k.conv1[0] = add_job(h, b, n + ".conv1.weight", co, cin, 3, 0, ca, taps_conv(3));
   if (cb) k.conv1[1] = add_job(h, b, n + ".conv1.weight", co, cin, 3, ca, cb, taps_conv(3));
   k.conv2 = add_job(h, b, n + ".conv2.weight", co, co, 3, 0, co, taps_conv(3));
-  if (cin == co) {
-    k.ident = add_ident(h, b, co);
-  } else {
+  if (cin != co) {
     k.shortcut[0] = add_job(h, b, n + ".conv_shortcut.weight", co, cin, 1, 0, ca, taps_conv(1));
     if (cb) k.shortcut[1] = add_job(h, b, n + ".conv_shortcut.weight", co, cin, 1, ca, cb, taps_conv(1));
     k.bias = add_bias(h, b, FusedBias::SUM2, co, n + ".conv2.bias", n + ".conv_shortcut.bias");
@@ -373,7 +364,6 @@
   add_job(h, b, n + ".to_v.weight", ch, ch, 1, 0, ch, taps_conv(1));
   k.out = add_job(h, b, n + ".to_out.0.weight", ch, ch, 1, 0, ch, taps_conv(1));
   k.bias = add_bias(h, b, FusedBias::QKV, (size_t)3 * ch, n + ".to_q.bias", n + ".to_k.bias", n + ".to_v.bias");
-  k.ident = add_ident(h, b, ch);
 }
 static void layout_transformer(NetBase* h, Bump& b, Block& k) {
   const std::string& n = k.name;
@@ -387,7 +377,6 @@
   k.ff1 = add_job(h, b, t + ".ff.net.0.proj.weight", 8 * c, c, 1, 0, c, taps_conv(1));
   k.ff2 = add_job(h, b, t + ".ff.net.2.weight", c, 4 * c, 1, 0, 4 * c, taps_conv(1));
   k.proj_out = add_job(h, b, n + ".proj_out.weight", c, c, 1, 0, c, taps_conv(1));
-  k.ident = add_ident(h, b, c);
 }
 static void layout_block(NetBase* h, Bump& b, Block& k) {
   switch (k.kind) {
@@ -424,7 +413,6 @@
     for (const PackJob& j : h->jobs) items.push_back(make_pack_item(h, j, h->packed));
     CK(launch_pack_batch(h->pack_batch, items, st));
   }
-  for (const auto& kv : h->ident_off) CK(launch_pack_identity(kv.first, (__nv_bfloat16*)(h->packed + kv.second), st));
   for (const FusedBias& f : h->fused) {
     float* dst = (float*)(h->packed + f.off);
     const int c = (int)h->params[f.p[0]].shape[0];
@@ -508,6 +496,10 @@
     set_seg(s, src, C / 8, C, H, W, PK<__nv_bfloat16>(woff), t);
   }
   void seg(ConvSeg& s, const Act& a, size_t woff, const TapSet& t) { seg(s, a.p, a.C, a.H, a.W, woff, t); }
+  static void residual(ConvParams& p, const Act& r) {
+    p.res = r.p;
+    p.res_img_stride = (long long)(r.C / 8) * make_geom(1, r.H, r.W).PL * 8;
+  }
 
   float2* gn_attach(const Act& a, const Act* b, const std::string& norm, float2* ss = nullptr, float eps = -1.f) {
     const int Ct = a.C + (b ? b->C : 0);
@@ -621,8 +613,7 @@
         }
         p.bias = PK<float>(k.bias);
       } else {
-        seg(p.seg[1], a, k.ident, taps_conv(1));
-        p.nseg = 2;
+        residual(p, a);
         p.bias = P(n + ".conv2.bias");
       }
       conv(p);
@@ -633,15 +624,12 @@
   }
 
   void linear(const Act& out, const Act& src, size_t woff, const float* bias, const float2* ss = nullptr,
-              const Act* residual = nullptr, size_t ident = 0, const float* vec = nullptr, int vec_stride = 0) {
+              const Act* res = nullptr, const float* vec = nullptr, int vec_stride = 0) {
     ConvParams p = conv_geom(N, out);
     p.nseg = 1;
     seg(p.seg[0], src, woff, taps_conv(1));
     if (ss) seg_norm(p.seg[0], ss, src.C, false);
-    if (residual) {
-      seg(p.seg[1], *residual, ident, taps_conv(1));
-      p.nseg = 2;
-    }
+    if (res) residual(p, *res);
     p.bias = bias;
     p.temb = vec; p.temb_stride = vec_stride;
     conv(p);
@@ -675,7 +663,7 @@
       return launch_mha_flash(q, o, N, C, heads, H, W, s, lse);
     });
     Act h2 = pooled("tf_h2", C, H, W, false);
-    linear(h2, ao, k.out, P(t + ".attn1.to_out.0.bias"), nullptr, &h0, k.ident, vec, C);
+    linear(h2, ao, k.out, P(t + ".attn1.to_out.0.bias"), nullptr, &h0, vec, C);
     Act n3 = pooled("tf_ln", C, H, W, false);
     layer_norm(h2, n3, t + ".norm3");
     Act ff1 = pooled("tf_ff1", 8 * C, H, W, false);
@@ -685,9 +673,9 @@
       return launch_geglu_pf8(x, y, N, 4 * C, H, W, s);
     });
     Act h3 = pooled("tf_h0", C, H, W, false);
-    linear(h3, gg, k.ff2, P(t + ".ff.net.2.bias"), nullptr, &h2, k.ident);
+    linear(h3, gg, k.ff2, P(t + ".ff.net.2.bias"), nullptr, &h2);
     Act out = output(k, C, H, W);
-    linear(out, h3, k.proj_out, P(n + ".proj_out.bias"), nullptr, &x, k.ident);
+    linear(out, h3, k.proj_out, P(n + ".proj_out.bias"), nullptr, &x);
     built->taps[n + ".attn2"] = h2;
     built->taps[n] = out;
     if (h->training) {
@@ -763,7 +751,7 @@
       });
     }
     Act out = output(k, C, H, W);
-    linear(out, ao, k.out, P(n + ".to_out.0.bias"), nullptr, &x, k.ident);
+    linear(out, ao, k.out, P(n + ".to_out.0.bias"), nullptr, &x);
     built->taps[n + ".qkv"] = qkv;
     built->taps[n + ".ao"] = ao;
     built->taps[n] = out;
diff --git a/audio_diffusion_b200/csrc/unet.cu b/audio_diffusion_b200/csrc/unet.cu
--- a/audio_diffusion_b200/csrc/unet.cu
+++ b/audio_diffusion_b200/csrc/unet.cu
@@ -190,12 +190,7 @@
     if (ops[i].kind == OP_CONV) {
       const ConvParams& p = ops[i].conv;
       double k = 0;
-      for (int s = 0; s < p.nseg; ++s) {
-        bool ident = false;
-        for (const auto& kv : h->ident_off)
-          if ((const uint8_t*)p.seg[s].wpack == h->packed + kv.second) ident = true;
-        if (!ident) k += (double)(p.up2 ? 9 : p.seg[s].ntaps) * p.seg[s].ksteps * 16;
-      }
+      for (int s = 0; s < p.nseg; ++s) k += (double)(p.up2 ? 9 : p.seg[s].ntaps) * p.seg[s].ksteps * 16;
       fl = 2.0 * p.N * p.H * p.W * p.cout * k;
     }
     op_flops[i] = fl;
@@ -221,6 +216,17 @@
   return n;
 }
 
+extern "C" int b200ad_unet_conv_residuals(const b200ad_unet* h, int N, int H, int W, int* res, int max_rows) {
+  const Plan pl = build_plan(h, nullptr, N, H, W);
+  int n = 0;
+  for (const Op& op : pl.lists[0].ops) {
+    if (op.kind != OP_CONV) continue;
+    if (n >= max_rows) return set_err("conv_residuals: more than %d conv launches", max_rows);
+    res[n++] = op.conv.res_img_stride != 0;
+  }
+  return n;
+}
+
 extern "C" int b200ad_unet_set_encoding(b200ad_unet* h, const float* enc, int S) {
   if (!h->cfg.cross_attention_dim) return set_err("set_encoding: this U-Net is unconditional");
   if (S < 1) return set_err("set_encoding: empty encoder sequence");
diff --git a/include/b200ad.h b/include/b200ad.h
--- a/include/b200ad.h
+++ b/include/b200ad.h
@@ -70,6 +70,7 @@
 
 #define B200AD_CONV_PLAN_COLS 12
 int b200ad_unet_conv_plan(const b200ad_unet* h, int N, int H, int W, int num_sms, int* rows, int max_rows);
+int b200ad_unet_conv_residuals(const b200ad_unet* h, int N, int H, int W, int* res, int max_rows);
 
 int b200ad_unet_set_training(b200ad_unet* h, int on);
 size_t b200ad_unet_grad_floats(b200ad_unet* h);
@@ -142,6 +143,10 @@
 int b200ad_gn_conv2d(const float* x, const float* gamma, const float* beta, int groups, float eps, int silu,
                      const float* w, const float* bias, float* y, int N, int cin, int cout, int H, int W, int K,
                      void* scratch, size_t scratch_bytes, void* stream);
+int b200ad_gn_conv2d_residual(const float* x, const float* gamma, const float* beta, int groups, float eps, int silu,
+                              const float* w, const float* bias, const float* temb, const float* residual, float* y,
+                              float* stats_out, int N, int cin, int cout, int H, int W, int K, void* scratch,
+                              size_t scratch_bytes, void* stream);
 int b200ad_conv2d_dgrad(const float* gy, const float* w, float* gx, int N, int cin, int cout, int H, int W, int K,
                         void* scratch, size_t scratch_bytes, void* stream);
 size_t b200ad_conv2d_wgrad_scratch_bytes(int N, int cin, int cout, int H, int W);
```

Result: faster. 0.9407, median of 6 (+1.2%).
